# binbinmeng/QCNN_GPU

Measured on NVIDIA B200. Metric: luma Mpixel/s (QVRCNN int8, 1080p), higher is better.
Workload: dtype int8

## Files before the change

### include/qvrcnn_b200.h

```cpp
#ifndef QVRCNN_B200_H
#define QVRCNN_B200_H

#include <stddef.h>
#include <stdint.h>

#ifdef __cplusplus
extern "C" {
#endif

#if defined(__GNUC__)
#define QV_API __attribute__((visibility("default")))
#else
#define QV_API
#endif

typedef struct qv_net qv_net;

enum {
    QV_OK = 0,
    QV_ERR_ARG = -1,
    QV_ERR_IO = -2,
    QV_ERR_CUDA = -3,
    QV_ERR_RANGE = -4,
    QV_ERR_STATE = -5
};

enum {
    QV_IMPL_AUTO = 0,
    QV_IMPL_LAYERED = 1,
    QV_IMPL_FUSED = 2
};

enum { QV_C1 = 0, QV_C2_1 = 1, QV_C2_2 = 2, QV_C3_1 = 3, QV_C3_2 = 4, QV_C4 = 5, QV_NLAYER = 6 };

QV_API const char *qv_last_error(void);
QV_API const char *qv_version(void);


QV_API int qv_create(int gpu_num, int batch, int channel, int height, int width, qv_net **out);
QV_API int qv_destroy(qv_net *net);

QV_API int qv_load_static_para(qv_net *net, const char *filename);
QV_API int qv_load_static_para_mem(qv_net *net, const void *image, size_t len);
QV_API int qv_load_static_para_hwcn(qv_net *net, const char *filename);

QV_API int qv_load_quant_params(qv_net *net, const char *filename);
QV_API int qv_read_quant_params(const char *filename, int32_t *out18);
QV_API int qv_set_weights(qv_net *net, int layer, const int8_t *w_kcrs, const int32_t *bias);
QV_API int qv_get_quant_params(const qv_net *net, int32_t *out18);

QV_API int qv_load_data(qv_net *net, const uint8_t *host_luma);
QV_API int qv_forward_blu(qv_net *net);
QV_API int qv_get_recon(qv_net *net, uint8_t *host_out);

QV_API int qv_forward_frames_host(qv_net *net, const uint8_t *h_in, uint8_t *h_out, int n_frames);
QV_API int qv_stream_yuv(qv_net *net, const char *anchor_yuv, const char *ori_yuv, const char *recon_yuv,
                         int first_frame, int n_frames, int64_t *sse_before, int64_t *sse_after);
QV_API int qv_stream_yuv_pf(qv_net *net, const char *anchor_yuv, const char *ori_yuv, const char *recon_yuv,
                            int first_frame, int n_frames, int64_t *sse_before_pf, int64_t *sse_after_pf);
QV_API int qv_forward_frames_device(qv_net *net, const uint8_t *d_in, uint8_t *d_out, int n_frames,
                                    void *cuda_stream);
QV_API int qv_forward_frames_device_sse(qv_net *net, const uint8_t *d_in, const uint8_t *d_ori, uint8_t *d_out,
                                        int n_frames, int64_t *d_sse, void *cuda_stream);
QV_API int qv_forward_rows_device(qv_net *net, const uint8_t *d_in, int img_height, int in_row0, int in_rows,
                                  uint8_t *d_out, int out_row0, int out_row1, void *cuda_stream);

QV_API int qv_synchronize(qv_net *net, void *cuda_stream);

typedef struct { unsigned char opaque[192]; } qv_strip_desc;
enum { QV_STRIP_ABOVE = 0, QV_STRIP_BELOW = 1 };
QV_API int qv_strip_setup(qv_net *net, int img_height, int row0, int row1);
QV_API int qv_strip_export(qv_net *net, qv_strip_desc *out);
QV_API int qv_strip_attach(qv_net *net, int side, const qv_strip_desc *neighbour);
QV_API int qv_strip_input(qv_net *net, int slot, void **d_rows);
QV_API int qv_strip_acquire(qv_net *net, int slot, void *cuda_stream);
QV_API int qv_strip_load(qv_net *net, int slot, const uint8_t *host_rows, void *cuda_stream);
QV_API int qv_strip_forward(qv_net *net, int slot, uint8_t *d_out, void *cuda_stream);
QV_API int qv_strip_forward_sse(qv_net *net, int slot, const uint8_t *d_ori_rows, uint8_t *d_out, int64_t *d_sse2,
                                void *cuda_stream);
QV_API int qv_strip_release(qv_net *net);

QV_API int qv_device_buffers(qv_net *net, void **d_x, void **d_x_rec);

QV_API int qv_sse_device(const uint8_t *d_a, const uint8_t *d_b, size_t n, int64_t *d_sse_accum, void *cuda_stream);

QV_API int qv_set_impl(qv_net *net, int impl);
QV_API int qv_get_impl(const qv_net *net);
QV_API long long qv_launch_count(const qv_net *net);
QV_API int qv_get_activation(qv_net *net, int which , int8_t *host_out);

QV_API int qv_debug_fused_tables(const void *model_image, size_t len, uint8_t *wimg, uint32_t *ops, int32_t *consts, size_t sizes[3]);

QV_API int qv_debug_fused_units(int sm_count, int n_frames, int height, int width, int row0, int row1, int row_window, int allow_line,
                                int32_t *units, size_t *n_units, int *grid);

QV_API int qv_convert_model_hwcn_to_vect_c(const char *file_in, const char *file_out);

QV_API int qv_solve_quant_params(const double *stepw_in, const double *blu_in, double *rows_out36);
QV_API int qv_write_quant_params_cpp(const char *filename, const double *rows36);
QV_API int qv_quantize_layer(const float *w, size_t n_w, const float *b, size_t n_b, double stepw, double ratio,
                             int8_t *w_q, int32_t *b_q);

QV_API void *qv_host_alloc(size_t bytes);
QV_API void qv_host_free(void *p);

QV_API int qv_yuv_read_luma(const char *filename, int frames, int height, int width, uint8_t *out);
QV_API int qv_yuv_read_frame(const char *filename, int n, int height, int width, uint8_t *out);
QV_API int qv_yuv_write_recon(const char *filename, const uint8_t *luma, int frames, int height, int width);
QV_API double qv_psnr(const uint8_t *data, const uint8_t *ori, size_t n, int64_t *sse_out);
QV_API double qv_psnr_from_sse(int64_t sse, size_t n);

#ifdef __cplusplus
}
#endif
#endif
```

### qcnn_gpu_b200/api.py

```python
from __future__ import annotations

import ctypes as C
import os
from typing import Optional

import numpy as np

_PKG = os.path.dirname(os.path.abspath(__file__))
LIB_PATH = os.environ.get("QVRCNN_B200_LIB", os.path.join(_PKG, "libqvrcnn_b200.so"))

IMPL_AUTO, IMPL_LAYERED, IMPL_FUSED = 0, 1, 2

ABI_SYMBOLS = (
    "qv_last_error", "qv_version", "qv_create", "qv_destroy", "qv_load_static_para",
    "qv_load_static_para_mem", "qv_load_static_para_hwcn", "qv_load_quant_params", "qv_read_quant_params",
    "qv_set_weights", "qv_get_quant_params", "qv_load_data", "qv_forward_blu", "qv_get_recon",
    "qv_forward_frames_host", "qv_stream_yuv", "qv_stream_yuv_pf", "qv_forward_frames_device", "qv_forward_frames_device_sse", "qv_forward_rows_device", "qv_device_buffers",
    "qv_sse_device", "qv_host_alloc", "qv_host_free",
    "qv_set_impl", "qv_get_impl", "qv_launch_count", "qv_get_activation",
    "qv_convert_model_hwcn_to_vect_c", "qv_yuv_read_luma", "qv_yuv_read_frame", "qv_yuv_write_recon",
    "qv_psnr", "qv_psnr_from_sse", "qv_solve_quant_params", "qv_write_quant_params_cpp", "qv_quantize_layer",
    "qv_debug_fused_tables", "qv_debug_fused_units", "qv_synchronize",
    "qv_strip_setup", "qv_strip_export", "qv_strip_attach", "qv_strip_input", "qv_strip_acquire", "qv_strip_load",
    "qv_strip_forward", "qv_strip_forward_sse", "qv_strip_release",
)

CUDA_STREAM_LEGACY = 1
STRIP_ABOVE, STRIP_BELOW = 0, 1
STRIP_DESC_BYTES = 192


def stream_arg(stream: int):
    return CUDA_STREAM_LEGACY if not stream else stream


class QVError(RuntimeError):
    def __init__(self, code: int, msg: str):
        super().__init__("qvrcnn_b200 error %d: %s" % (code, msg))
        self.code = code


_lib = None


def lib():
    global _lib
    if _lib is None:
        if not os.path.exists(LIB_PATH):
            raise ImportError("%s not found: build it with `python -c 'import __graft_entry__ as g; g.build()'` "
                              "(there is no fallback implementation)" % LIB_PATH)
        L = C.CDLL(LIB_PATH)
        vp, i32, cp = C.c_void_p, C.c_int, C.c_char_p
        L.qv_last_error.restype = cp
        L.qv_version.restype = cp
        L.qv_create.argtypes = [i32, i32, i32, i32, i32, C.POINTER(vp)]
        L.qv_destroy.argtypes = [vp]
        L.qv_load_static_para.argtypes = [vp, cp]
        L.qv_load_static_para_mem.argtypes = [vp, vp, C.c_size_t]
        L.qv_load_static_para_hwcn.argtypes = [vp, cp]
        L.qv_load_quant_params.argtypes = [vp, cp]
        L.qv_read_quant_params.argtypes = [cp, vp]
        L.qv_set_weights.argtypes = [vp, i32, vp, vp]
        L.qv_get_quant_params.argtypes = [vp, vp]
        L.qv_load_data.argtypes = [vp, vp]
        L.qv_forward_blu.argtypes = [vp]
        L.qv_get_recon.argtypes = [vp, vp]
        L.qv_forward_frames_host.argtypes = [vp, vp, vp, i32]
        L.qv_forward_frames_device.argtypes = [vp, vp, vp, i32, vp]
        L.qv_forward_frames_device_sse.argtypes = [vp, vp, vp, vp, i32, vp, vp]
        L.qv_host_alloc.argtypes = [C.c_size_t]
        L.qv_host_alloc.restype = vp
        L.qv_host_free.argtypes = [vp]
        L.qv_host_free.restype = None
        L.qv_stream_yuv.argtypes = [vp, cp, cp, cp, i32, i32, C.POINTER(C.c_int64), C.POINTER(C.c_int64)]
        L.qv_stream_yuv_pf.argtypes = [vp, cp, cp, cp, i32, i32, vp, vp]
        L.qv_forward_rows_device.argtypes = [vp, vp, i32, i32, i32, vp, i32, i32, vp]
        L.qv_sse_device.argtypes = [vp, vp, C.c_size_t, vp, vp]
        L.qv_set_impl.argtypes = [vp, i32]
        L.qv_get_impl.argtypes = [vp]
        L.qv_launch_count.argtypes = [vp]
        L.qv_launch_count.restype = C.c_longlong
        L.qv_get_activation.argtypes = [vp, i32, vp]
        L.qv_convert_model_hwcn_to_vect_c.argtypes = [cp, cp]
        L.qv_yuv_read_luma.argtypes = [cp, i32, i32, i32, vp]
        L.qv_yuv_read_frame.argtypes = [cp, i32, i32, i32, vp]
        L.qv_yuv_write_recon.argtypes = [cp, vp, i32, i32, i32]
        L.qv_psnr.argtypes = [vp, vp, C.c_size_t, C.POINTER(C.c_int64)]
        L.qv_psnr.restype = C.c_double
        L.qv_psnr_from_sse.argtypes = [C.c_int64, C.c_size_t]
        L.qv_psnr_from_sse.restype = C.c_double
        L.qv_solve_quant_params.argtypes = [vp, vp, vp]
        L.qv_write_quant_params_cpp.argtypes = [cp, vp]
        L.qv_quantize_layer.argtypes = [vp, C.c_size_t, vp, C.c_size_t, C.c_double, C.c_double, vp, vp]
        L.qv_synchronize.argtypes = [vp, vp]
        L.qv_strip_setup.argtypes = [vp, i32, i32, i32]
        L.qv_strip_export.argtypes = [vp, vp]
        L.qv_strip_attach.argtypes = [vp, i32, vp]
        L.qv_strip_input.argtypes = [vp, i32, C.POINTER(vp)]
        L.qv_strip_acquire.argtypes = [vp, i32, vp]
        L.qv_strip_load.argtypes = [vp, i32, vp, vp]
        L.qv_strip_forward.argtypes = [vp, i32, vp, vp]
        L.qv_strip_forward_sse.argtypes = [vp, i32, vp, vp, vp, vp]
        L.qv_strip_release.argtypes = [vp]
        _lib = L
    return _lib


def _check(rc: int) -> None:
    if rc != 0:
        raise QVError(rc, lib().qv_last_error().decode("utf-8", "replace"))


def _b(path) -> bytes:
    return os.fsencode(path)


class QVRCNN:

    def __init__(self, gpu_num: int, batch: int, channel: int, height: int, width: int):
        self._h = C.c_void_p()
        self.batch, self.channel, self.height, self.width = batch, channel, height, width
        _check(lib().qv_create(gpu_num, batch, channel, height, width, C.byref(self._h)))

    def close(self) -> None:
        if getattr(self, "_h", None) and self._h.value:
            lib().qv_destroy(self._h)
            self._h = C.c_void_p()

    __del__ = close

    def load_static_para(self, filename) -> int:
        _check(lib().qv_load_static_para(self._h, _b(filename)))
        return 0

    def load_static_para_mem(self, image: bytes) -> int:
        _check(lib().qv_load_static_para_mem(self._h, image, len(image)))
        return 0

    def load_static_para_hwcn(self, filename) -> int:
        _check(lib().qv_load_static_para_hwcn(self._h, _b(filename)))
        return 0

    def load_quant_params(self, filename) -> int:
        _check(lib().qv_load_quant_params(self._h, _b(filename)))
        return 0

    def set_weights(self, layer: int, w_kcrs: np.ndarray, bias: np.ndarray) -> int:
        w = np.ascontiguousarray(w_kcrs, np.int8)
        b = np.ascontiguousarray(bias, np.int32)
        _check(lib().qv_set_weights(self._h, layer, w.ctypes.data, b.ctypes.data))
        return 0

    def quant_params(self) -> np.ndarray:
        q = np.zeros(18, np.int32)
        _check(lib().qv_get_quant_params(self._h, q.ctypes.data))
        return q.reshape(6, 3)

    def load_data(self, input_u8: np.ndarray) -> int:
        x = np.ascontiguousarray(input_u8, np.uint8)
        assert x.size == self.batch * self.height * self.width, x.shape
        _check(lib().qv_load_data(self._h, x.ctypes.data))
        return 0

    def forward_blu(self) -> int:
        _check(lib().qv_forward_blu(self._h))
        return 0

    def get_recon(self) -> np.ndarray:
        out = np.empty((self.batch, self.height, self.width), np.uint8)
        _check(lib().qv_get_recon(self._h, out.ctypes.data))
        return out

    def forward_frames_host(self, frames_u8: np.ndarray, out: Optional[np.ndarray] = None) -> np.ndarray:
        x = np.ascontiguousarray(frames_u8, np.uint8)
        n = x.size // (self.height * self.width)
        if out is None:
            out = np.empty_like(x)
        _check(lib().qv_forward_frames_host(self._h, x.ctypes.data, out.ctypes.data, n))
        return out

    def stream_yuv(self, anchor_yuv: str, ori_yuv: Optional[str], recon_yuv: Optional[str], first_frame: int, n_frames: int):
        b, a = C.c_int64(0), C.c_int64(0)
        enc = lambda p: p.encode() if p else None
        _check(lib().qv_stream_yuv(self._h, enc(anchor_yuv), enc(ori_yuv), enc(recon_yuv), first_frame, n_frames,
                                   C.byref(b) if ori_yuv else None, C.byref(a) if ori_yuv else None))
        return int(b.value), int(a.value)

    def stream_yuv_pf(self, anchor_yuv: str, ori_yuv: str, recon_yuv: Optional[str], first_frame: int, n_frames: int):
        before = np.zeros(max(n_frames, 0), np.int64)
        after = np.zeros(max(n_frames, 0), np.int64)
        enc = lambda p: os.fsencode(p) if p else None
        _check(lib().qv_stream_yuv_pf(self._h, enc(anchor_yuv), enc(ori_yuv), enc(recon_yuv), first_frame, n_frames,
                                      before.ctypes.data, after.ctypes.data))
        return before, after

    def forward_frames_host_ptr(self, in_ptr: int, out_ptr: int, n: int) -> None:
        _check(lib().qv_forward_frames_host(self._h, in_ptr, out_ptr, n))

    def forward_frames_device(self, d_in: int, d_out: int, n: int, stream: int = 0) -> None:
        _check(lib().qv_forward_frames_device(self._h, d_in, d_out, n, stream or None))

    def forward_frames_device_sse(self, d_in: int, d_ori: int, d_out: int, n: int, d_sse: int, stream: int = 0) -> None:
        _check(lib().qv_forward_frames_device_sse(self._h, d_in, d_ori, d_out, n, d_sse, stream or None))

    def forward_rows_device(self, d_in: int, img_height: int, in_row0: int, in_rows: int, d_out: int,
                            out_row0: int, out_row1: int, stream: int = 0) -> None:
        _check(lib().qv_forward_rows_device(self._h, d_in, img_height, in_row0, in_rows, d_out, out_row0,
                                            out_row1, stream or None))

    def synchronize(self, stream: int = 0) -> None:
        _check(lib().qv_synchronize(self._h, stream or None))

    def strip_setup(self, img_height: int, row0: int, row1: int) -> None:
        _check(lib().qv_strip_setup(self._h, img_height, row0, row1))
        self._strip_bytes = (row1 - row0) * self.width

    def strip_export(self) -> bytes:
        buf = C.create_string_buffer(STRIP_DESC_BYTES)
        _check(lib().qv_strip_export(self._h, buf))
        return buf.raw

    def strip_attach(self, side: int, desc: bytes) -> None:
        assert len(desc) == STRIP_DESC_BYTES
        _check(lib().qv_strip_attach(self._h, side, C.create_string_buffer(desc, STRIP_DESC_BYTES)))

    def strip_input(self, slot: int) -> int:
        p = C.c_void_p()
        _check(lib().qv_strip_input(self._h, slot, C.byref(p)))
        return int(p.value)

    def strip_acquire(self, slot: int, stream: int = 0) -> None:
        _check(lib().qv_strip_acquire(self._h, slot, stream or None))

    def strip_load(self, slot: int, rows_u8: np.ndarray, stream: int = 0) -> None:
        x = np.ascontiguousarray(rows_u8, np.uint8)
        assert x.size == getattr(self, "_strip_bytes", -1), "strip_load: expected the %d bytes of this handle's rows, got %d" % (getattr(self, "_strip_bytes", -1), x.size)
        _check(lib().qv_strip_load(self._h, slot, x.ctypes.data, stream or None))

    def strip_forward(self, slot: int, d_out: int, stream: int = 0) -> None:
        _check(lib().qv_strip_forward(self._h, slot, d_out, stream or None))

    def strip_forward_sse(self, slot: int, d_ori_rows: int, d_out: int, d_sse2: int, stream: int = 0) -> None:
        _check(lib().qv_strip_forward_sse(self._h, slot, d_ori_rows, d_out, d_sse2, stream or None))

    def strip_release(self) -> None:
        _check(lib().qv_strip_release(self._h))

    def set_impl(self, impl: int) -> None:
        _check(lib().qv_set_impl(self._h, impl))

    def get_impl(self) -> int:
        return lib().qv_get_impl(self._h)

    def launch_count(self) -> int:
        return int(lib().qv_launch_count(self._h))

    def get_activation(self, which: int) -> np.ndarray:
        out = np.empty((64 if which == 1 else 48, self.height, self.width), np.int8)
        _check(lib().qv_get_activation(self._h, which, out.ctypes.data))
        return out


def sse_device(d_a: int, d_b: int, n: int, d_accum: int, stream: int = 0) -> None:
    _check(lib().qv_sse_device(d_a, d_b, n, d_accum, stream or None))


def read_quant_params(filename) -> np.ndarray:
    q = np.zeros(18, np.int32)
    _check(lib().qv_read_quant_params(_b(filename), q.ctypes.data))
    return q.reshape(6, 3)


def convert_model_hwcn_to_vect_c(file_in, file_out) -> None:
    _check(lib().qv_convert_model_hwcn_to_vect_c(_b(file_in), _b(file_out)))


def solve_quant_params(stepw_in, blu_in) -> np.ndarray:
    a = np.ascontiguousarray(stepw_in, np.float64)
    b = np.ascontiguousarray(blu_in, np.float64)
    assert a.size == 6 and b.size == 6
    out = np.zeros(36, np.float64)
    _check(lib().qv_solve_quant_params(a.ctypes.data, b.ctypes.data, out.ctypes.data))
    return out.reshape(6, 6)


def write_quant_params_cpp(filename, rows) -> None:
    r = np.ascontiguousarray(rows, np.float64)
    assert r.size == 36
    _check(lib().qv_write_quant_params_cpp(_b(filename), r.ctypes.data))


def quantize_layer(w: np.ndarray, b: np.ndarray, stepw: float, ratio: float):
    wf = np.ascontiguousarray(w, np.float32)
    bf = np.ascontiguousarray(b, np.float32)
    wq = np.empty(wf.shape, np.int8)
    bq = np.empty(bf.shape, np.int32)
    _check(lib().qv_quantize_layer(wf.ctypes.data, wf.size, bf.ctypes.data, bf.size, float(stepw), float(ratio), wq.ctypes.data, bq.ctypes.data))
    return wq, bq


def psnr_from_sse(sse: int, n: int) -> float:
    return float(lib().qv_psnr_from_sse(sse, n))


class VRCNNData:

    def __init__(self, frame: int, height: int, width: int):
        self.frame, self.h, self.w = frame, height, width
        self.nSize = frame * height * width
        self.ori = np.zeros((frame, height, width), np.uint8)
        self.input = np.zeros((frame, height, width), np.uint8)
        self.recon = np.zeros((frame, height, width), np.uint8)

    def read_data(self, orifile, inputfile) -> int:
        _check(lib().qv_yuv_read_luma(_b(orifile), self.frame, self.h, self.w, self.ori.ctypes.data))
        _check(lib().qv_yuv_read_luma(_b(inputfile), self.frame, self.h, self.w, self.input.ctypes.data))
        return 0

    def read_frame(self, orifile, inputfile, n: int) -> int:
        self.frame = 1
        _check(lib().qv_yuv_read_frame(_b(orifile), n, self.h, self.w, self.ori.ctypes.data))
        _check(lib().qv_yuv_read_frame(_b(inputfile), n, self.h, self.w, self.input.ctypes.data))
        return 0

    def psnr(self, data: np.ndarray) -> float:
        d = np.ascontiguousarray(data, np.uint8)
        return float(lib().qv_psnr(d.ctypes.data, self.ori.ctypes.data, self.nSize, None))

    def save_recon_as(self, filename) -> int:
        _check(lib().qv_yuv_write_recon(_b(filename), self.recon.ctypes.data, self.frame, self.h, self.w))
        return 0
```

### qcnn_gpu_b200/csrc/qv_api.cu

```cuda
#include <algorithm>
#include <atomic>
#include <condition_variable>
#include <cstdio>
#include <cstdlib>
#include <cstring>
#include <mutex>
#include <random>
#include <thread>
#include <vector>

#include <fcntl.h>
#include <unistd.h>

#include <cuda_runtime.h>

#include "qv_fused.h"
#include "qv_internal.h"
#include "qv_layered.h"

using namespace qv;

#define QV_CUDA(expr)                                                                       \
    do {                                                                                    \
        cudaError_t e__ = (expr);                                                           \
        if (e__ != cudaSuccess) {                                                           \
            set_error("%s failed: %s (%s:%d)", #expr, cudaGetErrorString(e__), __FILE__, __LINE__); \
            return QV_ERR_CUDA;                                                             \
        }                                                                                   \
    } while (0)

namespace {
constexpr int STRIP_HALO = 6;
constexpr size_t STRIP_HDR = 256, STRIP_PUB = 0, STRIP_DONE = 64, STRIP_CTR = 128;
constexpr uint32_t STRIP_MAGIC = 0x51565354u;
struct StripDescImpl {
    uint32_t magic;
    int32_t dev, row0, row1, width, img_h;
    uint64_t nonce;
    uint64_t base, slot_off, slot_stride;
    uint64_t net;
    cudaIpcMemHandle_t ipc;
    char pci[16];
};
static_assert(sizeof(StripDescImpl) <= sizeof(qv_strip_desc), "qv_strip_desc too small");
struct StripPeer {
    bool attached = false, ipc = false, same_device = false;
    uint8_t *base = nullptr;
    qv_net *net = nullptr;
    StripDescImpl d{};
};
struct StripState {
    bool on = false;
    int img_h = 0, row0 = 0, row1 = 0;
    uint8_t *block = nullptr;
    size_t slot_stride = 0;
    uint32_t seq = 0, slot_seq[2] = {0, 0};
    uint32_t fills[2] = {0, 0}, forwards[2] = {0, 0};
    cudaStream_t last_stream = nullptr;
    bool used = false;
    StripPeer peer[2];
};
std::mutex g_strip_mu;
std::vector<qv_net *> g_strip_nets[64];
uint64_t process_nonce()
{
    static const uint64_t n = [] {
        std::random_device rd;
        return ((uint64_t)rd() << 32) ^ (uint64_t)rd() ^ ((uint64_t)getpid() << 17);
    }();
    return n;
}
}

struct qv_net {
    StripState strip;
    int dev = 0, batch = 0, H = 0, W = 0;
    cudaStream_t st = nullptr;
    cudaStream_t pst[2] = {nullptr, nullptr};
    cudaEvent_t ev_compute = nullptr;
    uint8_t *d_x = nullptr, *d_rec = nullptr;
    uint8_t *d_slot_in[2] = {nullptr, nullptr}, *d_slot_out[2] = {nullptr, nullptr};
    uint8_t *h_pin_in[2] = {nullptr, nullptr}, *h_pin_out[2] = {nullptr, nullptr};
    int8_t *d_a1 = nullptr, *d_a2 = nullptr, *d_a3 = nullptr;
    int act_frames = 0;
    uint8_t *d_rows_tmp = nullptr;
    size_t rows_tmp_bytes = 0;
    ModelHost model;
    LayeredModel lm;
    FusedModel *fm = nullptr;
    bool uploaded = false;
    int impl = QV_IMPL_AUTO;
    long long launches = 0;
};

static int set_device(const qv_net *net) { QV_CUDA(cudaSetDevice(net->dev)); return QV_OK; }

static void free_layered(qv_net *net)
{
    for (int l = 0; l < QV_NLAYER; ++l) {
        cudaFree(net->lm.L[l].d_wpk);
        cudaFree(net->lm.L[l].d_bias);
        net->lm.L[l].d_wpk = nullptr;
        net->lm.L[l].d_bias = nullptr;
    }
}

static inline int pack4(const int8_t *p, int stride, int n)
{
    int v = 0;
    for (int j = 0; j < n; ++j) v |= ((int)(uint8_t)p[j * stride]) << (8 * j);
    return v;
}

static int upload_layered(qv_net *net)
{
    free_layered(net);
    for (int l = 0; l < QV_NLAYER; ++l) {
        const LayerShape &s = kLayers[l];
        const LayerHost &L = net->model.L[l];
        std::vector<int32_t> wpk;
        const int R = s.k;
        if (l == QV_C1) {
            wpk.assign(5 * 64 * 2, 0);
            for (int r = 0; r < 5; ++r)
                for (int k = 0; k < 64; ++k) {
                    const int8_t *row = &L.w[((size_t)k * 5 + r) * 5];
                    wpk[(r * 64 + k) * 2 + 0] = pack4(row, 1, 4);
                    wpk[(r * 64 + k) * 2 + 1] = pack4(row + 4, 1, 1);
                }
        } else if (l == QV_C4) {
            wpk.assign(9 * 12, 0);
            for (int t = 0; t < 9; ++t)
                for (int c4 = 0; c4 < 12; ++c4)
                    wpk[t * 12 + c4] = pack4(&L.w[((size_t)(4 * c4) * 3 + t / 3) * 3 + t % 3], 9, 4);
        } else {
            const int C4 = s.cin / 4, G = s.cout / 16;
            wpk.assign((size_t)G * R * R * C4 * 16, 0);
            for (int g = 0; g < G; ++g)
                for (int t = 0; t < R * R; ++t)
                    for (int c4 = 0; c4 < C4; ++c4)
                        for (int j = 0; j < 16; ++j) {
                            const int k = g * 16 + j;
                            wpk[(((size_t)g * R * R + t) * C4 + c4) * 16 + j] =
                                pack4(&L.w[(((size_t)k * s.cin + 4 * c4) * R + t / R) * R + t % R], R * R, 4);
                        }
        }
        LayeredLayer &D = net->lm.L[l];
        D.cout = s.cout;
        D.q.blu = L.blu; D.q.mul = L.mul; D.q.shift = L.shift;
        D.q.rbias = (1 << (L.shift - 1)) / L.mul;
        QV_CUDA(cudaMalloc(&D.d_wpk, wpk.size() * sizeof(int32_t)));
        QV_CUDA(cudaMalloc(&D.d_bias, L.b.size() * sizeof(int32_t)));
        QV_CUDA(cudaMemcpyAsync(D.d_wpk, wpk.data(), wpk.size() * sizeof(int32_t), cudaMemcpyHostToDevice, net->st));
        QV_CUDA(cudaMemcpyAsync(D.d_bias, L.b.data(), L.b.size() * sizeof(int32_t), cudaMemcpyHostToDevice, net->st));
        QV_CUDA(cudaStreamSynchronize(net->st));
    }
    net->lm.c4_bias = net->model.L[QV_C4].b[0];
    return QV_OK;
}

static int validate_qparams(const ModelHost &m)
{
    for (int l = 0; l < QV_NLAYER; ++l) {
        const LayerHost &L = m.L[l];
        if (L.mul <= 0 || L.shift < 1 || L.shift > 30) {
            set_error("layer %d: mul=%d shift=%d outside the supported range (mul>0, 1<=shift<=30)", l, L.mul, L.shift);
            return QV_ERR_RANGE;
        }
        if (l != QV_C4 && (L.blu < 0 || L.blu >= (1 << 24))) {
            set_error("layer %d: blu=%d outside [0, 2^24)", l, L.blu);
            return QV_ERR_RANGE;
        }
    }
    return QV_OK;
}

static int sync_model(qv_net *net)
{
    net->uploaded = false;
    if (!net->model.complete()) return QV_OK;
    int rc = validate_qparams(net->model);
    if (rc) return rc;
    rc = check_fp32_exact_envelope(net->model);
    if (rc) return rc;
    if ((rc = set_device(net))) return rc;
    if ((rc = upload_layered(net))) return rc;
    if (net->fm) { fused_free(net->fm); net->fm = nullptr; }
    net->fm = fused_upload(net->model, net->st);
    net->uploaded = true;
    return QV_OK;
}

static int ensure_acts(qv_net *net)
{
    if (net->d_a1) return QV_OK;
    int frames = std::min(net->batch, 8);
    const size_t px = (size_t)frames * net->H * net->W;
    QV_CUDA(cudaMalloc(&net->d_a1, px * 64));
    QV_CUDA(cudaMalloc(&net->d_a2, px * 48));
    QV_CUDA(cudaMalloc(&net->d_a3, px * 48));
    net->act_frames = frames;
    return QV_OK;
}

static int run_forward(qv_net *net, const uint8_t *d_in, uint8_t *d_out, int n, int H, int W, cudaStream_t st,
                       const uint8_t *d_ori = nullptr, int64_t *d_sse = nullptr)
{
    if (!net->uploaded) {
        set_error("forward called before a complete model (weights + quant params) was loaded");
        return QV_ERR_STATE;
    }
    int impl = net->impl;
    if (impl == QV_IMPL_AUTO) impl = net->fm ? QV_IMPL_FUSED : QV_IMPL_LAYERED;
    if (impl == QV_IMPL_FUSED) {
        if (!net->fm) { set_error("fused tcgen05 path is not available in this build"); return QV_ERR_STATE; }
        if (d_sse && H > FUSED_SSE_MAX_H) { set_error("per-frame SSE: frame height %d exceeds %d", H, FUSED_SSE_MAX_H); return QV_ERR_ARG; }
        QV_CUDA(fused_forward(net->fm, d_in, d_out, n, H, W, st, &net->launches, nullptr, d_ori, d_sse));
        return QV_OK;
    }
    int rc = ensure_acts(net);
    if (rc) return rc;
    const size_t cap_px = (size_t)net->act_frames * net->H * net->W;
    const size_t fpx = (size_t)H * W;
    if (fpx > cap_px) { set_error("frame of %dx%d exceeds the handle's activation scratch", W, H); return QV_ERR_ARG; }
    const int chunk = (int)std::max<size_t>(1, cap_px / fpx);
    for (int f0 = 0; f0 < n; f0 += chunk) {
        const int c = std::min(chunk, n - f0);
        QV_CUDA(layered_forward(net->lm, d_in + (size_t)f0 * fpx, d_out + (size_t)f0 * fpx, c, H, W, net->d_a1,
                                net->d_a2, net->d_a3, st, &net->launches));
    }
    if (d_sse) {
        for (int f = 0; f < n; ++f) {
            const size_t o = (size_t)f * fpx;
            QV_CUDA(sse_accumulate(d_in + o, d_ori + o, fpx, d_sse + 2 * f, st));
            QV_CUDA(sse_accumulate(d_out + o, d_ori + o, fpx, d_sse + 2 * f + 1, st));
        }
        net->launches += 2 * n;
    }
    return QV_OK;
}

extern "C" {

int qv_create(int gpu_num, int batch, int channel, int height, int width, qv_net **out)
{
    if (!out) { set_error("qv_create: null output pointer"); return QV_ERR_ARG; }
    *out = nullptr;
    if (channel != 1) { set_error("qv_create: channel must be 1 (luma), got %d", channel); return QV_ERR_ARG; }
    if (batch < 1 || height < 1 || width < 1) { set_error("qv_create: bad geometry %dx%dx%d", batch, height, width); return QV_ERR_ARG; }
    int ndev = 0;
    if (cudaGetDeviceCount(&ndev) != cudaSuccess || ndev == 0) {
        set_error("qv_create: no CUDA device (this library has no CPU fallback)");
        return QV_ERR_CUDA;
    }
    if (gpu_num < 0 || gpu_num >= ndev) { set_error("qv_create: gpu_num %d out of range (%d devices)", gpu_num, ndev); return QV_ERR_ARG; }
    QV_CUDA(cudaSetDevice(gpu_num));
    qv_net *net = new qv_net();
    net->dev = gpu_num; net->batch = batch; net->H = height; net->W = width;
    const size_t bytes = (size_t)batch * height * width;
    cudaError_t e = cudaStreamCreateWithFlags(&net->st, cudaStreamNonBlocking);
    if (e == cudaSuccess) e = cudaMalloc(&net->d_x, bytes);
    if (e == cudaSuccess) e = cudaMalloc(&net->d_rec, bytes);
    if (e != cudaSuccess) {
        set_error("qv_create: %s", cudaGetErrorString(e));
        qv_destroy(net);
        return QV_ERR_CUDA;
    }
    *out = net;
    return QV_OK;
}

int qv_destroy(qv_net *net)
{
    if (!net) return QV_OK;
    cudaSetDevice(net->dev);
    if (net->st) cudaStreamSynchronize(net->st);
    qv_strip_release(net);
    free_layered(net);
    if (net->fm) fused_free(net->fm);
    cudaFree(net->d_x); cudaFree(net->d_rec);
    cudaFree(net->d_a1); cudaFree(net->d_a2); cudaFree(net->d_a3);
    cudaFree(net->d_rows_tmp);
    for (int i = 0; i < 2; ++i) {
        cudaFree(net->d_slot_in[i]); cudaFree(net->d_slot_out[i]);
        cudaFreeHost(net->h_pin_in[i]); cudaFreeHost(net->h_pin_out[i]);
        if (net->pst[i]) cudaStreamDestroy(net->pst[i]);
    }
    if (net->ev_compute) cudaEventDestroy(net->ev_compute);
    if (net->st) cudaStreamDestroy(net->st);
    delete net;
    return QV_OK;
}

int qv_load_static_para_mem(qv_net *net, const void *image, size_t len)
{
    if (!net || !image) { set_error("qv_load_static_para_mem: null argument"); return QV_ERR_ARG; }
    ModelHost m;
    int rc = parse_model_vect_c((const uint8_t *)image, len, m);
    if (rc) return rc;
    net->model = m;
    return sync_model(net);
}

int qv_debug_fused_tables(const void *image, size_t len, uint8_t *wimg, uint32_t *ops, int32_t *consts, size_t sizes[3])
{
    if (!image || !sizes) { set_error("qv_debug_fused_tables: null argument"); return QV_ERR_ARG; }
    ModelHost m;
    int rc = parse_model_vect_c((const uint8_t *)image, len, m);
    if (rc) return rc;
    std::vector<uint8_t> w;
    std::vector<uint32_t> o;
    std::vector<int32_t> c;
    fused_debug_tables(m, w, o, c);
    if (wimg && sizes[0] >= w.size()) memcpy(wimg, w.data(), w.size());
    if (ops && sizes[1] >= o.size()) memcpy(ops, o.data(), o.size() * sizeof(uint32_t));
    if (consts && sizes[2] >= c.size()) memcpy(consts, c.data(), c.size() * sizeof(int32_t));
    sizes[0] = w.size(); sizes[1] = o.size(); sizes[2] = c.size();
    return QV_OK;
}

int qv_debug_fused_units(int sm_count, int n_frames, int height, int width, int row0, int row1, int row_window, int allow_line,
                         int32_t *units, size_t *n_units, int *grid)
{
    if (!n_units || !grid) { set_error("qv_debug_fused_units: null argument"); return QV_ERR_ARG; }
    std::vector<int> u;
    int g = 0;
    if (fused_debug_units(sm_count, n_frames, height, width, row0, row1, row_window != 0, allow_line != 0, u, g)) {
        set_error("qv_debug_fused_units: bad geometry");
        return QV_ERR_ARG;
    }
    if (units && *n_units >= u.size() / 5) memcpy(units, u.data(), u.size() * sizeof(int));
    *n_units = u.size() / 5;
    *grid = g;
    return QV_OK;
}

int qv_load_static_para(qv_net *net, const char *filename)
{
    if (!net) { set_error("qv_load_static_para: null handle"); return QV_ERR_ARG; }
    std::vector<uint8_t> buf;
    int rc = read_file(filename, buf);
    if (rc) { set_error("cannot open model file. (%s)", filename ? filename : "(null)"); return rc; }
    return qv_load_static_para_mem(net, buf.data(), buf.size());
}

int qv_load_static_para_hwcn(qv_net *net, const char *filename)
{
    if (!net) { set_error("qv_load_static_para_hwcn: null handle"); return QV_ERR_ARG; }
    std::vector<uint8_t> buf;
    int rc = read_file(filename, buf);
    if (rc) return rc;
    ModelHost m;
    rc = parse_model_hwcn(buf.data(), buf.size(), m);
    if (rc) return rc;
    net->model = m;
    return sync_model(net);
}

int qv_load_quant_params(qv_net *net, const char *filename)
{
    if (!net) { set_error("qv_load_quant_params: null handle"); return QV_ERR_ARG; }
    int32_t q[18];
    int rc = qv_read_quant_params(filename, q);
    if (rc) return rc;
    for (int l = 0; l < QV_NLAYER; ++l) {
        LayerHost &L = net->model.L[l];
        L.blu = q[3 * l]; L.mul = q[3 * l + 1]; L.shift = q[3 * l + 2];
        L.have_q = true;
    }
    return sync_model(net);
}

int qv_set_weights(qv_net *net, int layer, const int8_t *w_kcrs, const int32_t *bias)
{
    if (!net || !w_kcrs || !bias || layer < 0 || layer >= QV_NLAYER) { set_error("qv_set_weights: bad argument"); return QV_ERR_ARG; }
    const LayerShape &s = kLayers[layer];
    LayerHost &L = net->model.L[layer];
    L.w.assign(w_kcrs, w_kcrs + (size_t)s.cout * s.cin * s.k * s.k);
    L.b.assign(bias, bias + s.cout);
    L.have_w = true;
    return sync_model(net);
}

int qv_get_quant_params(const qv_net *net, int32_t *out18)
{
    if (!net || !out18) { set_error("qv_get_quant_params: null argument"); return QV_ERR_ARG; }
    for (int l = 0; l < QV_NLAYER; ++l) {
        out18[3 * l] = net->model.L[l].blu; out18[3 * l + 1] = net->model.L[l].mul; out18[3 * l + 2] = net->model.L[l].shift;
    }
    return QV_OK;
}

int qv_load_data(qv_net *net, const uint8_t *host_luma)
{
    if (!net || !host_luma) { set_error("qv_load_data: null argument"); return QV_ERR_ARG; }
    int rc = set_device(net);
    if (rc) return rc;
    const size_t bytes = (size_t)net->batch * net->H * net->W;
    QV_CUDA(cudaMemcpyAsync(net->d_x, host_luma, bytes, cudaMemcpyHostToDevice, net->st));
    QV_CUDA(cudaStreamSynchronize(net->st));
    return QV_OK;
}

static int kernel_report(qv_net *net)
{
    const int f = net->fm ? fused_take_failure(net->fm) : 0;
    if (!f) return QV_OK;
    set_error(f == 2 ? "fused kernel: a CTA saw other shared-memory / TMEM bases than the operand table was built for"
              : f == 3 ? "strip mode: a neighbour GPU's rows were never published (the frame data of this call is not valid)"
                       : "fused kernel: an mbarrier wait timed out (the frame data of this call is not valid)");
    return QV_ERR_CUDA;
}

int qv_forward_blu(qv_net *net)
{
    if (!net) { set_error("qv_forward_blu: null handle"); return QV_ERR_ARG; }
    int rc = set_device(net);
    if (rc) return rc;
    rc = run_forward(net, net->d_x, net->d_rec, net->batch, net->H, net->W, net->st);
    if (rc) return rc;
    QV_CUDA(cudaStreamSynchronize(net->st));
    return kernel_report(net);
}

int qv_get_recon(qv_net *net, uint8_t *host_out)
{
    if (!net || !host_out) { set_error("qv_get_recon: null argument"); return QV_ERR_ARG; }
    int rc = set_device(net);
    if (rc) return rc;
    const size_t bytes = (size_t)net->batch * net->H * net->W;
    QV_CUDA(cudaMemcpyAsync(host_out, net->d_rec, bytes, cudaMemcpyDeviceToHost, net->st));
    QV_CUDA(cudaStreamSynchronize(net->st));
    return kernel_report(net);
}

int qv_forward_frames_device(qv_net *net, const uint8_t *d_in, uint8_t *d_out, int n_frames, void *cuda_stream)
{
    if (!net || !d_in || !d_out || n_frames < 0) { set_error("qv_forward_frames_device: bad argument"); return QV_ERR_ARG; }
    int rc = set_device(net);
    if (rc) return rc;
    cudaStream_t st = cuda_stream ? (cudaStream_t)cuda_stream : net->st;
    if (n_frames > 0) {
        rc = run_forward(net, d_in, d_out, n_frames, net->H, net->W, st);
        if (rc) return rc;
    }
    if (!cuda_stream) { QV_CUDA(cudaStreamSynchronize(st)); return kernel_report(net); }
    return QV_OK;
}

int qv_forward_frames_device_sse(qv_net *net, const uint8_t *d_in, const uint8_t *d_ori, uint8_t *d_out, int n_frames,
                                 int64_t *d_sse, void *cuda_stream)
{
    if (!net || !d_in || !d_ori || !d_out || !d_sse || n_frames < 0) { set_error("qv_forward_frames_device_sse: bad argument"); return QV_ERR_ARG; }
    int rc = set_device(net);
    if (rc) return rc;
    cudaStream_t st = cuda_stream ? (cudaStream_t)cuda_stream : net->st;
    if (n_frames > 0) {
        rc = run_forward(net, d_in, d_out, n_frames, net->H, net->W, st, d_ori, d_sse);
        if (rc) return rc;
    }
    if (!cuda_stream) { QV_CUDA(cudaStreamSynchronize(st)); return kernel_report(net); }
    return QV_OK;
}

int qv_forward_rows_device(qv_net *net, const uint8_t *d_in, int img_height, int in_row0, int in_rows, uint8_t *d_out,
                           int out_row0, int out_row1, void *cuda_stream)
{
    if (!net || !d_in || !d_out) { set_error("qv_forward_rows_device: null argument"); return QV_ERR_ARG; }
    const int in_row1 = in_row0 + in_rows;
    if (img_height < 1 || in_row0 < 0 || in_rows < 1 || in_row1 > img_height || out_row0 < in_row0 || out_row1 > in_row1 ||
        out_row0 > out_row1) { set_error("qv_forward_rows_device: inconsistent row ranges"); return QV_ERR_ARG; }
    if ((in_row0 != 0 && out_row0 - in_row0 < STRIP_HALO) || (in_row1 != img_height && in_row1 - out_row1 < STRIP_HALO)) {
        set_error("qv_forward_rows_device: need 6 halo rows on every interior strip edge");
        return QV_ERR_ARG;
    }
    int rc = set_device(net);
    if (rc) return rc;
    cudaStream_t st = cuda_stream ? (cudaStream_t)cuda_stream : net->st;
    const size_t W = net->W;
    const bool fused_path = net->impl == QV_IMPL_FUSED || (net->impl == QV_IMPL_AUTO && net->fm);
    if (fused_path) {
        if (!net->uploaded || !net->fm) { set_error("forward called before a complete model (weights + quant params) was loaded"); return QV_ERR_STATE; }
        FusedRows fr;
        fr.own0 = in_row0; fr.own1 = in_row1; fr.out0 = out_row0; fr.out1 = out_row1;
        QV_CUDA(fused_forward(net->fm, d_in, d_out, 1, img_height, net->W, st, &net->launches, &fr));
    } else {
        const size_t need = (size_t)in_rows * W;
        if (need > (size_t)net->batch * net->H * net->W) {
            set_error("qv_forward_rows_device: window larger than the handle's geometry");
            return QV_ERR_ARG;
        }
        if (net->rows_tmp_bytes < need) {
            QV_CUDA(cudaStreamSynchronize(st));
            cudaFree(net->d_rows_tmp);
            net->d_rows_tmp = nullptr; net->rows_tmp_bytes = 0;
            QV_CUDA(cudaMalloc(&net->d_rows_tmp, need));
            net->rows_tmp_bytes = need;
        }
        rc = run_forward(net, d_in, net->d_rows_tmp, 1, in_rows, net->W, st);
        if (rc) return rc;
        QV_CUDA(cudaMemcpyAsync(d_out, net->d_rows_tmp + (size_t)(out_row0 - in_row0) * W, (size_t)(out_row1 - out_row0) * W,
                                cudaMemcpyDeviceToDevice, st));
    }
    if (!cuda_stream) { QV_CUDA(cudaStreamSynchronize(st)); return kernel_report(net); }
    return QV_OK;
}

int qv_synchronize(qv_net *net, void *cuda_stream)
{
    if (!net) { set_error("qv_synchronize: null handle"); return QV_ERR_ARG; }
    int rc = set_device(net);
    if (rc) return rc;
    QV_CUDA(cudaStreamSynchronize(cuda_stream ? (cudaStream_t)cuda_stream : net->st));
    return kernel_report(net);
}

static void strip_detach(qv_net *net)
{
    for (StripPeer &p : net->strip.peer) {
        if (p.attached && p.ipc && p.base) cudaIpcCloseMemHandle(p.base);
        p = StripPeer{};
    }
}

int qv_strip_release(qv_net *net)
{
    if (!net) { set_error("qv_strip_release: null handle"); return QV_ERR_ARG; }
    if (!net->strip.on) return QV_OK;
    cudaSetDevice(net->dev);
    cudaStreamSynchronize(net->st);
    strip_detach(net);
    cudaFree(net->strip.block);
    net->strip = StripState{};
    if (net->dev >= 0 && net->dev < 64) {
        std::lock_guard<std::mutex> l(g_strip_mu);
        auto &v = g_strip_nets[net->dev];
        v.erase(std::remove(v.begin(), v.end(), net), v.end());
    }
    return QV_OK;
}

int qv_strip_setup(qv_net *net, int img_height, int row0, int row1)
{
    if (!net) { set_error("qv_strip_setup: null handle"); return QV_ERR_ARG; }
    if (img_height < 1 || row0 < 0 || row1 <= row0 || row1 > img_height) { set_error("qv_strip_setup: rows [%d, %d) of %d", row0, row1, img_height); return QV_ERR_ARG; }
    int rc = set_device(net);
    if (rc) return rc;
    qv_strip_release(net);
    StripState &S = net->strip;
    S.img_h = img_height; S.row0 = row0; S.row1 = row1;
    S.slot_stride = ((size_t)(row1 - row0) * net->W + 255) / 256 * 256;
    QV_CUDA(cudaMalloc(&S.block, STRIP_HDR + 2 * S.slot_stride));
    QV_CUDA(cudaMemset(S.block, 0, STRIP_HDR));
    QV_CUDA(cudaDeviceSynchronize());
    S.on = true;
    if (net->dev >= 0 && net->dev < 64) {
        std::lock_guard<std::mutex> l(g_strip_mu);
        g_strip_nets[net->dev].push_back(net);
    }
    return QV_OK;
}

int qv_strip_export(qv_net *net, qv_strip_desc *out)
{
    if (!net || !out) { set_error("qv_strip_export: null argument"); return QV_ERR_ARG; }
    if (!net->strip.on) { set_error("qv_strip_export: qv_strip_setup has not been called"); return QV_ERR_STATE; }
    int rc = set_device(net);
    if (rc) return rc;
    StripDescImpl d{};
    d.magic = STRIP_MAGIC; d.dev = net->dev; d.row0 = net->strip.row0; d.row1 = net->strip.row1; d.width = net->W; d.img_h = net->strip.img_h;
    d.nonce = process_nonce();
    d.base = (uint64_t)(uintptr_t)net->strip.block; d.slot_off = STRIP_HDR; d.slot_stride = net->strip.slot_stride;
    d.net = (uint64_t)(uintptr_t)net;
    QV_CUDA(cudaIpcGetMemHandle(&d.ipc, net->strip.block));
    QV_CUDA(cudaDeviceGetPCIBusId(d.pci, (int)sizeof(d.pci), net->dev));
    memset(out, 0, sizeof(*out));
    memcpy(out, &d, sizeof(d));
    return QV_OK;
}

int qv_strip_attach(qv_net *net, int side, const qv_strip_desc *neighbour)
{
    if (!net || !neighbour || (side != QV_STRIP_ABOVE && side != QV_STRIP_BELOW)) { set_error("qv_strip_attach: bad argument"); return QV_ERR_ARG; }
    StripState &S = net->strip;
    if (!S.on) { set_error("qv_strip_attach: qv_strip_setup has not been called"); return QV_ERR_STATE; }
    StripDescImpl d;
    memcpy(&d, neighbour, sizeof(d));
    if (d.magic != STRIP_MAGIC) { set_error("qv_strip_attach: not a strip descriptor"); return QV_ERR_ARG; }
    if (d.width != net->W || d.img_h != S.img_h) { set_error("qv_strip_attach: the neighbour's frame is %dx%d, this one %dx%d", d.width, d.img_h, net->W, S.img_h); return QV_ERR_ARG; }
    if (side == QV_STRIP_ABOVE ? d.row1 != S.row0 : d.row0 != S.row1) {
        set_error("qv_strip_attach: rows [%d, %d) are not adjacent %s rows [%d, %d)", d.row0, d.row1, side == QV_STRIP_ABOVE ? "above" : "below", S.row0, S.row1);
        return QV_ERR_ARG;
    }
    if (d.row1 - d.row0 < STRIP_HALO) {
        set_error("qv_strip_attach: the neighbour holds %d rows, fewer than the %d-row halo (use fewer strips)", d.row1 - d.row0, STRIP_HALO);
        return QV_ERR_ARG;
    }
    int rc = set_device(net);
    if (rc) return rc;
    StripPeer &P = S.peer[side];
    if (P.attached && P.ipc && P.base) cudaIpcCloseMemHandle(P.base);
    P = StripPeer{};
    if (d.nonce == process_nonce()) {
        if (d.dev != net->dev) {
            int can = 0;
            QV_CUDA(cudaDeviceCanAccessPeer(&can, net->dev, d.dev));
            if (!can) { set_error("qv_strip_attach: device %d cannot map memory of device %d (no peer access)", net->dev, d.dev); return QV_ERR_CUDA; }
            cudaError_t e = cudaDeviceEnablePeerAccess(d.dev, 0);
            if (e == cudaErrorPeerAccessAlreadyEnabled) { cudaGetLastError(); e = cudaSuccess; }
            QV_CUDA(e);
        }
        P.base = (uint8_t *)(uintptr_t)d.base;
        P.net = (qv_net *)(uintptr_t)d.net;
    } else {
        char my_pci[16] = {0};
        QV_CUDA(cudaDeviceGetPCIBusId(my_pci, (int)sizeof(my_pci), net->dev));
        if (strncmp(my_pci, d.pci, sizeof(my_pci)) == 0) {
            set_error("qv_strip_attach: the neighbour strip belongs to another process on the SAME GPU; strips of different processes must be on different GPUs");
            return QV_ERR_ARG;
        }
        void *p = nullptr;
        QV_CUDA(cudaIpcOpenMemHandle(&p, d.ipc, cudaIpcMemLazyEnablePeerAccess));
        P.base = (uint8_t *)p;
        P.ipc = true;
    }
    P.d = d;
    char my_pci[16] = {0};
    QV_CUDA(cudaDeviceGetPCIBusId(my_pci, (int)sizeof(my_pci), net->dev));
    P.same_device = strncmp(my_pci, d.pci, sizeof(my_pci)) == 0;
    P.attached = true;
    return QV_OK;
}

int qv_strip_input(qv_net *net, int slot, void **d_rows)
{
    if (!net || !d_rows || slot < 0 || slot > 1) { set_error("qv_strip_input: bad argument"); return QV_ERR_ARG; }
    if (!net->strip.on) { set_error("qv_strip_input: qv_strip_setup has not been called"); return QV_ERR_STATE; }
    *d_rows = net->strip.block + STRIP_HDR + (size_t)slot * net->strip.slot_stride;
    return QV_OK;
}

static int check_shared_device_stream(qv_net *net, cudaStream_t st, const char *who)
{
    std::lock_guard<std::mutex> l(g_strip_mu);
    for (qv_net *o : g_strip_nets[net->dev])
        if (o != net && o->strip.used && o->strip.last_stream != st) {
            set_error("%s: several strips live on GPU %d: drive all of them on ONE caller-provided stream (kernels of different launches "
                      "must not wait for each other on one GPU, so stream order is what orders them)", who, net->dev);
            return QV_ERR_STATE;
        }
    return QV_OK;
}

int qv_strip_acquire(qv_net *net, int slot, void *cuda_stream)
{
    if (!net || slot < 0 || slot > 1) { set_error("qv_strip_acquire: bad argument"); return QV_ERR_ARG; }
    StripState &S = net->strip;
    if (!S.on) { set_error("qv_strip_acquire: qv_strip_setup has not been called"); return QV_ERR_STATE; }
    int rc = set_device(net);
    if (rc) return rc;
    cudaStream_t st = cuda_stream ? (cudaStream_t)cuda_stream : net->st;
    if ((rc = check_shared_device_stream(net, st, "qv_strip_acquire"))) return rc;
    S.last_stream = st; S.used = true;
    const uint32_t s = S.slot_seq[slot];
    const uint32_t *w[2] = {nullptr, nullptr};
    for (int side = 0; side < 2; ++side) {
        const StripPeer &P = S.peer[side];
        if (!P.attached || s == 0) continue;
        if (P.same_device) {
            if (P.net->strip.forwards[slot] < S.forwards[slot]) {
                set_error("qv_strip_acquire: the neighbour strip on the same GPU has not yet consumed slot %d (issue the strips' calls frame by frame)", slot);
                return QV_ERR_STATE;
            }
        } else {
            w[side] = reinterpret_cast<const uint32_t *>(P.base + STRIP_DONE);
        }
    }
    if (net->fm && (w[0] || w[1])) {
        QV_CUDA(fused_wait_words(net->fm, w[0], s, w[1], s, st));
        net->launches += 1;
    }
    S.fills[slot] += 1;
    return QV_OK;
}

int qv_strip_load(qv_net *net, int slot, const uint8_t *host_rows, void *cuda_stream)
{
    if (!host_rows) { set_error("qv_strip_load: null argument"); return QV_ERR_ARG; }
    int rc = qv_strip_acquire(net, slot, cuda_stream);
    if (rc) return rc;
    StripState &S = net->strip;
    QV_CUDA(cudaMemcpyAsync(S.block + STRIP_HDR + (size_t)slot * S.slot_stride, host_rows, (size_t)(S.row1 - S.row0) * net->W,
                            cudaMemcpyHostToDevice, cuda_stream ? (cudaStream_t)cuda_stream : net->st));
    return QV_OK;
}

static int strip_forward(qv_net *net, int slot, const uint8_t *d_ori, uint8_t *d_out, int64_t *d_sse, void *cuda_stream, const char *who)
{
    StripState &S = net->strip;
    if (!S.on) { set_error("%s: qv_strip_setup has not been called", who); return QV_ERR_STATE; }
    if (!net->uploaded || !net->fm || net->impl == QV_IMPL_LAYERED) {
        set_error("%s: needs a loaded model and the fused path (peer-mapped halo rows are read by the fused kernel)", who);
        return QV_ERR_STATE;
    }
    if ((S.row0 > 0 && !S.peer[QV_STRIP_ABOVE].attached) || (S.row1 < S.img_h && !S.peer[QV_STRIP_BELOW].attached)) {
        set_error("%s: rows [%d, %d) of %d have an interior edge with no neighbour attached", who, S.row0, S.row1, S.img_h);
        return QV_ERR_STATE;
    }
    if (d_sse && S.img_h > FUSED_SSE_MAX_H) { set_error("%s: frame height %d exceeds %d", who, S.img_h, FUSED_SSE_MAX_H); return QV_ERR_ARG; }
    int rc = set_device(net);
    if (rc) return rc;
    cudaStream_t st = cuda_stream ? (cudaStream_t)cuda_stream : net->st;
    if ((rc = check_shared_device_stream(net, st, who))) return rc;
    const size_t W = net->W;
    FusedRows fr;
    fr.own0 = fr.out0 = S.row0; fr.own1 = fr.out1 = S.row1;
    fr.pub = reinterpret_cast<uint32_t *>(S.block + STRIP_PUB);
    fr.done = reinterpret_cast<uint32_t *>(S.block + STRIP_DONE);
    fr.done_ctr = reinterpret_cast<uint32_t *>(S.block + STRIP_CTR);
    for (int side = 0; side < 2; ++side) {
        if (side == QV_STRIP_ABOVE ? S.row0 == 0 : S.row1 == S.img_h) continue;
        const StripPeer &P = S.peer[side];
        const uint8_t *rows = P.base + P.d.slot_off + (size_t)slot * P.d.slot_stride;
        const uint32_t *flag = reinterpret_cast<const uint32_t *>(P.base + STRIP_PUB);
        if (P.same_device) {
            if (P.net->strip.fills[slot] == 0) {
                set_error("%s: the neighbour strip on the same GPU has not filled slot %d yet (strips that share a GPU: all loads of a frame, then its forwards, on one stream)", who, slot);
                return QV_ERR_STATE;
            }
            flag = nullptr;
        }
        if (side == QV_STRIP_ABOVE) { fr.top_rows = STRIP_HALO; fr.d_top = rows + (size_t)(P.d.row1 - P.d.row0 - STRIP_HALO) * W; fr.flag_top = flag; }
        else { fr.bot_rows = STRIP_HALO; fr.d_bot = rows; fr.flag_bot = flag; }
    }
    const uint32_t seq = ++S.seq;
    S.slot_seq[slot] = seq;
    S.forwards[slot] += 1;
    S.last_stream = st; S.used = true;
    fr.seq = seq;
    const uint8_t *own = S.block + STRIP_HDR + (size_t)slot * S.slot_stride;
    QV_CUDA(fused_forward(net->fm, own, d_out, 1, S.img_h, net->W, st, &net->launches, &fr, d_ori, d_sse));
    if (!cuda_stream) { QV_CUDA(cudaStreamSynchronize(st)); return kernel_report(net); }
    return QV_OK;
}

int qv_strip_forward(qv_net *net, int slot, uint8_t *d_out, void *cuda_stream)
{
    if (!net || !d_out || slot < 0 || slot > 1) { set_error("qv_strip_forward: bad argument"); return QV_ERR_ARG; }
    return strip_forward(net, slot, nullptr, d_out, nullptr, cuda_stream, "qv_strip_forward");
}

int qv_strip_forward_sse(qv_net *net, int slot, const uint8_t *d_ori_rows, uint8_t *d_out, int64_t *d_sse2, void *cuda_stream)
{
    if (!net || !d_ori_rows || !d_out || !d_sse2 || slot < 0 || slot > 1) { set_error("qv_strip_forward_sse: bad argument"); return QV_ERR_ARG; }
    return strip_forward(net, slot, d_ori_rows, d_out, d_sse2, cuda_stream, "qv_strip_forward_sse");
}

int qv_forward_frames_host(qv_net *net, const uint8_t *h_in, uint8_t *h_out, int n_frames)
{
    if (!net || !h_in || !h_out || n_frames < 0) { set_error("qv_forward_frames_host: bad argument"); return QV_ERR_ARG; }
    int rc = set_device(net);
    if (rc) return rc;
    const size_t fpx = (size_t)net->H * net->W;
    std::vector<int> chunks;
    {
        static const int num[10] = {1, 3, 4, 8, 16, 16, 8, 4, 3, 1};
        int left = n_frames;
        if (n_frames >= 16) {
            for (int k = 0; k < 10 && left > 0; ++k) {
                int want = k == 9 ? left : std::max(1, n_frames * num[k] / 64);
                while (want > 0 && left > 0) {
                    const int c = std::min(std::min(want, left), net->batch);
                    chunks.push_back(c); want -= c; left -= c;
                }
            }
        }
        const char *ov = getenv("QV_E2E_CHUNKS");
        if (ov && *ov) {
            chunks.clear(); left = n_frames;
            for (const char *p = ov; *p && left > 0;) {
                const int c = std::min(std::min(std::max(1, atoi(p)), left), net->batch);
                chunks.push_back(c); left -= c;
                while (*p && *p != ',') ++p;
                if (*p == ',') ++p;
            }
        }
        const int uni = std::max(1, std::min(net->batch, (n_frames + 3) / 4));
        while (left > 0) { const int c = std::min(uni, left); chunks.push_back(c); left -= c; }
    }
    const size_t cbytes = (size_t)net->batch * fpx;
    cudaPointerAttributes ai{}, ao{};
    bool pinned_in = cudaPointerGetAttributes(&ai, h_in) == cudaSuccess && ai.type == cudaMemoryTypeHost;
    bool pinned_out = cudaPointerGetAttributes(&ao, h_out) == cudaSuccess && ao.type == cudaMemoryTypeHost;
    cudaGetLastError();
    if (!net->ev_compute) QV_CUDA(cudaEventCreateWithFlags(&net->ev_compute, cudaEventDisableTiming));
    for (int i = 0; i < 2; ++i) {
        if (!net->pst[i]) QV_CUDA(cudaStreamCreateWithFlags(&net->pst[i], cudaStreamNonBlocking));
        if (!net->d_slot_in[i]) QV_CUDA(cudaMalloc(&net->d_slot_in[i], cbytes));
        if (!net->d_slot_out[i]) QV_CUDA(cudaMalloc(&net->d_slot_out[i], cbytes));
        if (!pinned_in && !net->h_pin_in[i]) QV_CUDA(cudaMallocHost(&net->h_pin_in[i], cbytes));
        if (!pinned_out && !net->h_pin_out[i]) QV_CUDA(cudaMallocHost(&net->h_pin_out[i], cbytes));
    }
    struct Pending { int f0 = -1, c = 0; } pend[2];
    auto drain = [&](int s) -> int {
        if (pend[s].f0 < 0) return QV_OK;
        QV_CUDA(cudaStreamSynchronize(net->pst[s]));
        if (!pinned_out) memcpy(h_out + (size_t)pend[s].f0 * fpx, net->h_pin_out[s], (size_t)pend[s].c * fpx);
        pend[s].f0 = -1;
        return QV_OK;
    };
    int slot = 0;
    int f0 = 0;
    for (size_t ci = 0; ci < chunks.size(); f0 += chunks[ci], ++ci, slot ^= 1) {
        const int c = chunks[ci];
        const size_t bytes = (size_t)c * fpx;
        if ((rc = drain(slot))) return rc;
        const uint8_t *src = h_in + (size_t)f0 * fpx;
        if (!pinned_in) { memcpy(net->h_pin_in[slot], src, bytes); src = net->h_pin_in[slot]; }
        QV_CUDA(cudaMemcpyAsync(net->d_slot_in[slot], src, bytes, cudaMemcpyHostToDevice, net->pst[slot]));
        const bool fused_path = net->impl == QV_IMPL_FUSED || (net->impl == QV_IMPL_AUTO && net->fm);
        if (f0 > 0 && !fused_path) QV_CUDA(cudaStreamWaitEvent(net->pst[slot], net->ev_compute, 0));
        rc = run_forward(net, net->d_slot_in[slot], net->d_slot_out[slot], c, net->H, net->W, net->pst[slot]);
        if (rc) return rc;
        QV_CUDA(cudaEventRecord(net->ev_compute, net->pst[slot]));
        uint8_t *dst = pinned_out ? h_out + (size_t)f0 * fpx : net->h_pin_out[slot];
        QV_CUDA(cudaMemcpyAsync(dst, net->d_slot_out[slot], bytes, cudaMemcpyDeviceToHost, net->pst[slot]));
        pend[slot].f0 = f0; pend[slot].c = c;
    }
    if ((rc = drain(0))) return rc;
    if ((rc = drain(1))) return rc;
    return kernel_report(net);
}

namespace {
struct StreamSlot {
    uint8_t *h_in = nullptr, *h_ori = nullptr, *h_out = nullptr;
    uint8_t *d_in = nullptr, *d_ori = nullptr, *d_out = nullptr;
    cudaStream_t st = nullptr;
    cudaEvent_t done = nullptr;
    int state = 0;
    int f0 = 0, c = 0;
};
struct StreamShared {
    std::mutex mu;
    std::condition_variable cv;
    bool failed = false;
    char msg[256] = {0};
    void fail(const char *m) { std::lock_guard<std::mutex> l(mu); if (!failed) { failed = true; snprintf(msg, sizeof(msg), "%s", m); } cv.notify_all(); }
};
bool read_luma(FILE *f, long long frame, size_t fpx, uint8_t *dst)
{
    if (fseeko(f, (off_t)(frame * (long long)(fpx + fpx / 2)), SEEK_SET) != 0) return false;
    return fread(dst, 1, fpx, f) == fpx;
}
}

int qv_stream_yuv_pf(qv_net *net, const char *anchor_yuv, const char *ori_yuv, const char *recon_yuv, int first_frame, int n_frames,
                     int64_t *sse_before_pf, int64_t *sse_after_pf)
{
    if (!net || !anchor_yuv || first_frame < 0 || n_frames < 0) { set_error("qv_stream_yuv_pf: bad argument"); return QV_ERR_ARG; }
    if ((sse_before_pf || sse_after_pf) && !ori_yuv) { set_error("qv_stream_yuv_pf: an SSE was asked for but no original file given"); return QV_ERR_ARG; }
    int rc = set_device(net);
    if (rc) return rc;
    for (int j = 0; j < n_frames; ++j) {
        if (sse_before_pf) sse_before_pf[j] = 0;
        if (sse_after_pf) sse_after_pf[j] = 0;
    }
    if (n_frames == 0) return QV_OK;
    const size_t fpx = (size_t)net->H * net->W;
    const int C = net->batch, NS = 3;
    FILE *fa = fopen(anchor_yuv, "rb"), *fo = ori_yuv ? fopen(ori_yuv, "rb") : nullptr, *fr = nullptr;
    if (!fa) { set_error("open file failed. (%s)", anchor_yuv); return QV_ERR_IO; }
    if (ori_yuv && !fo) { fclose(fa); set_error("open file failed. (%s)", ori_yuv); return QV_ERR_IO; }
    if (recon_yuv) {
        const int fd = open(recon_yuv, O_CREAT | O_RDWR, 0644);
        fr = fd >= 0 ? fdopen(fd, "r+b") : nullptr;
        if (!fr && fd >= 0) close(fd);
        if (!fr) { fclose(fa); if (fo) fclose(fo); set_error("open file failed. (%s)", recon_yuv); return QV_ERR_IO; }
    }
    StreamSlot slot[3];
    StreamShared sh;
    int64_t *d_sse = nullptr;
    const size_t sse_bytes = (size_t)n_frames * 2 * sizeof(int64_t);
    cudaError_t e = cudaMalloc(&d_sse, sse_bytes);
    if (e == cudaSuccess) e = cudaMemset(d_sse, 0, sse_bytes);
    for (int s = 0; s < NS && e == cudaSuccess; ++s) {
        StreamSlot &S = slot[s];
        e = cudaMallocHost(&S.h_in, C * fpx);
        if (e == cudaSuccess) e = cudaMallocHost(&S.h_out, C * fpx);
        if (e == cudaSuccess && fo) e = cudaMallocHost(&S.h_ori, C * fpx);
        if (e == cudaSuccess) e = cudaMalloc(&S.d_in, C * fpx);
        if (e == cudaSuccess) e = cudaMalloc(&S.d_out, C * fpx);
        if (e == cudaSuccess && fo) e = cudaMalloc(&S.d_ori, C * fpx);
        if (e == cudaSuccess) e = cudaStreamCreateWithFlags(&S.st, cudaStreamNonBlocking);
        if (e == cudaSuccess) e = cudaEventCreateWithFlags(&S.done, cudaEventDisableTiming);
    }
    const int nchunk = (n_frames + C - 1) / C;
    auto cleanup = [&]() {
        for (int s = 0; s < NS; ++s) {
            StreamSlot &S = slot[s];
            if (S.st) cudaStreamSynchronize(S.st);
            cudaFreeHost(S.h_in); cudaFreeHost(S.h_out); cudaFreeHost(S.h_ori);
            cudaFree(S.d_in); cudaFree(S.d_out); cudaFree(S.d_ori);
            if (S.done) cudaEventDestroy(S.done);
            if (S.st) cudaStreamDestroy(S.st);
        }
        cudaFree(d_sse);
        fclose(fa); if (fo) fclose(fo); if (fr) fclose(fr);
    };
    if (e != cudaSuccess) { cleanup(); set_error("qv_stream_yuv: %s", cudaGetErrorString(e)); return QV_ERR_CUDA; }

    std::thread reader([&] {
        for (int k = 0; k < nchunk; ++k) {
            StreamSlot &S = slot[k % NS];
            {
                std::unique_lock<std::mutex> l(sh.mu);
                sh.cv.wait(l, [&] { return S.state == 0 || sh.failed; });
                if (sh.failed) return;
            }
            const int f0 = k * C, c = std::min(C, n_frames - f0);
            for (int j = 0; j < c; ++j) {
                if (!read_luma(fa, (long long)first_frame + f0 + j, fpx, S.h_in + (size_t)j * fpx) ||
                    (fo && !read_luma(fo, (long long)first_frame + f0 + j, fpx, S.h_ori + (size_t)j * fpx))) {
                    sh.fail("qv_stream_yuv: short read (file smaller than the requested frame range)");
                    return;
                }
            }
            { std::lock_guard<std::mutex> l(sh.mu); S.f0 = f0; S.c = c; S.state = 1; }
            sh.cv.notify_all();
        }
    });
    const int dev = net->dev;
    std::thread writer([&] {
        cudaSetDevice(dev);
        std::vector<uint8_t> zeros(fpx / 2, 0);
        for (int k = 0; k < nchunk; ++k) {
            StreamSlot &S = slot[k % NS];
            {
                std::unique_lock<std::mutex> l(sh.mu);
                sh.cv.wait(l, [&] { return S.state == 2 || sh.failed; });
                if (sh.failed) return;
            }
            if (cudaEventSynchronize(S.done) != cudaSuccess) { sh.fail("qv_stream_yuv: the GPU stage failed"); return; }
            if (fr) {
                bool ok = fseeko(fr, (off_t)(((long long)first_frame + S.f0) * (long long)(fpx + fpx / 2)), SEEK_SET) == 0;
                for (int j = 0; j < S.c && ok; ++j)
                    ok = fwrite(S.h_out + (size_t)j * fpx, 1, fpx, fr) == fpx && fwrite(zeros.data(), 1, fpx / 2, fr) == fpx / 2;
                if (!ok) { sh.fail("qv_stream_yuv: write to the reconstruction file failed"); return; }
            }
            { std::lock_guard<std::mutex> l(sh.mu); S.state = 0; }
            sh.cv.notify_all();
        }
    });
    const bool fused_path = net->impl == QV_IMPL_FUSED || (net->impl == QV_IMPL_AUTO && net->fm);
    cudaEvent_t ev_compute = nullptr;
    if (!fused_path && cudaEventCreateWithFlags(&ev_compute, cudaEventDisableTiming) != cudaSuccess) {
        sh.fail("qv_stream_yuv: the GPU stage failed");
        rc = QV_ERR_CUDA;
    }
    for (int k = 0; k < nchunk && rc == QV_OK; ++k) {
        StreamSlot &S = slot[k % NS];
        {
            std::unique_lock<std::mutex> l(sh.mu);
            sh.cv.wait(l, [&] { return S.state == 1 || sh.failed; });
            if (sh.failed) break;
        }
        const size_t bytes = (size_t)S.c * fpx;
        e = cudaMemcpyAsync(S.d_in, S.h_in, bytes, cudaMemcpyHostToDevice, S.st);
        if (e == cudaSuccess && fo) e = cudaMemcpyAsync(S.d_ori, S.h_ori, bytes, cudaMemcpyHostToDevice, S.st);
        if (e == cudaSuccess && !fused_path && k > 0) e = cudaStreamWaitEvent(S.st, ev_compute, 0);
        if (e == cudaSuccess) {
            rc = run_forward(net, S.d_in, S.d_out, S.c, net->H, net->W, S.st, fo ? S.d_ori : nullptr, fo ? d_sse + 2 * (size_t)S.f0 : nullptr);
            if (rc == QV_OK && !fused_path) e = cudaEventRecord(ev_compute, S.st);
        }
        if (e == cudaSuccess && rc == QV_OK) e = cudaMemcpyAsync(S.h_out, S.d_out, bytes, cudaMemcpyDeviceToHost, S.st);
        if (e == cudaSuccess && rc == QV_OK) e = cudaEventRecord(S.done, S.st);
        if (e != cudaSuccess) { set_error("qv_stream_yuv: %s", cudaGetErrorString(e)); rc = QV_ERR_CUDA; }
        if (rc != QV_OK) { sh.fail("qv_stream_yuv: the GPU stage failed"); break; }
        { std::lock_guard<std::mutex> l(sh.mu); S.state = 2; }
        sh.cv.notify_all();
    }
    reader.join();
    writer.join();
    if (ev_compute) { for (int s = 0; s < NS; ++s) cudaStreamSynchronize(slot[s].st); cudaEventDestroy(ev_compute); }
    std::vector<int64_t> h_sse(fo ? (size_t)n_frames * 2 : 0);
    if (rc == QV_OK && !sh.failed) {
        for (int s = 0; s < NS; ++s) cudaStreamSynchronize(slot[s].st);
        if (fo && cudaMemcpy(h_sse.data(), d_sse, sse_bytes, cudaMemcpyDeviceToHost) != cudaSuccess) {
            set_error("qv_stream_yuv_pf: copy of the SSEs failed");
            rc = QV_ERR_CUDA;
        }
    }
    cleanup();
    if (rc == QV_OK && sh.failed) { set_error("%s", sh.msg); rc = strstr(sh.msg, "GPU") ? QV_ERR_CUDA : QV_ERR_IO; }
    if (rc != QV_OK) return rc;
    for (int j = 0; fo && j < n_frames; ++j) {
        if (sse_before_pf) sse_before_pf[j] = h_sse[2 * (size_t)j];
        if (sse_after_pf) sse_after_pf[j] = h_sse[2 * (size_t)j + 1];
    }
    return kernel_report(net);
}

int qv_stream_yuv(qv_net *net, const char *anchor_yuv, const char *ori_yuv, const char *recon_yuv, int first_frame, int n_frames,
                  int64_t *sse_before, int64_t *sse_after)
{
    if (!net || !anchor_yuv || first_frame < 0 || n_frames < 0) { set_error("qv_stream_yuv: bad argument"); return QV_ERR_ARG; }
    if ((sse_before || sse_after) && !ori_yuv) { set_error("qv_stream_yuv: an SSE was asked for but no original file given"); return QV_ERR_ARG; }
    std::vector<int64_t> before(ori_yuv ? n_frames : 0), after(ori_yuv ? n_frames : 0);
    const int rc = qv_stream_yuv_pf(net, anchor_yuv, ori_yuv, recon_yuv, first_frame, n_frames, ori_yuv ? before.data() : nullptr,
                                    ori_yuv ? after.data() : nullptr);
    if (sse_before) *sse_before = 0;
    if (sse_after) *sse_after = 0;
    if (rc != QV_OK) return rc;
    for (size_t j = 0; j < before.size(); ++j) {
        if (sse_before) *sse_before += before[j];
        if (sse_after) *sse_after += after[j];
    }
    return QV_OK;
}

void *qv_host_alloc(size_t bytes)
{
    if (bytes == 0) bytes = 1;
    void *p = nullptr;
    int ndev = 0;
    if (cudaGetDeviceCount(&ndev) == cudaSuccess && ndev > 0 && cudaHostAlloc(&p, bytes, cudaHostAllocPortable) == cudaSuccess) return p;
    cudaGetLastError();
    return malloc(bytes);
}

void qv_host_free(void *p)
{
    if (!p) return;
    cudaPointerAttributes a{};
    if (cudaPointerGetAttributes(&a, p) == cudaSuccess && a.type == cudaMemoryTypeHost) { cudaFreeHost(p); return; }
    cudaGetLastError();
    free(p);
}

int qv_device_buffers(qv_net *net, void **d_x, void **d_x_rec)
{
    if (!net) { set_error("qv_device_buffers: null handle"); return QV_ERR_ARG; }
    if (d_x) *d_x = net->d_x;
    if (d_x_rec) *d_x_rec = net->d_rec;
    return QV_OK;
}

int qv_sse_device(const uint8_t *d_a, const uint8_t *d_b, size_t n, int64_t *d_sse_accum, void *cuda_stream)
{
    if (!d_a || !d_b || !d_sse_accum) { set_error("qv_sse_device: null argument"); return QV_ERR_ARG; }
    if (n == 0) return QV_OK;
    QV_CUDA(sse_accumulate(d_a, d_b, n, d_sse_accum, (cudaStream_t)cuda_stream));
    return QV_OK;
}

int qv_set_impl(qv_net *net, int impl)
{
    if (!net || impl < QV_IMPL_AUTO || impl > QV_IMPL_FUSED) { set_error("qv_set_impl: bad argument"); return QV_ERR_ARG; }
    net->impl = impl;
    return QV_OK;
}

int qv_get_impl(const qv_net *net)
{
    if (!net) return QV_ERR_ARG;
    if (net->impl != QV_IMPL_AUTO) return net->impl;
    return net->fm ? QV_IMPL_FUSED : QV_IMPL_LAYERED;
}

long long qv_launch_count(const qv_net *net) { return net ? net->launches : 0; }

int qv_get_activation(qv_net *net, int which, int8_t *host_out)
{
    if (!net || !host_out || which < 1 || which > 3) { set_error("qv_get_activation: bad argument"); return QV_ERR_ARG; }
    if (!net->d_a1) { set_error("qv_get_activation: the layered path has not run on this handle"); return QV_ERR_STATE; }
    int rc = set_device(net);
    if (rc) return rc;
    const int C = which == 1 ? 64 : 48;
    const int8_t *src = which == 1 ? net->d_a1 : (which == 2 ? net->d_a2 : net->d_a3);
    const size_t HW = (size_t)net->H * net->W;
    int8_t *tmp = nullptr;
    QV_CUDA(cudaMalloc(&tmp, HW * C));
    cudaError_t e = nhwc_to_planar(src, tmp, C, HW, net->st);
    if (e == cudaSuccess) e = cudaMemcpyAsync(host_out, tmp, HW * C, cudaMemcpyDeviceToHost, net->st);
    if (e == cudaSuccess) e = cudaStreamSynchronize(net->st);
    cudaFree(tmp);
    QV_CUDA(e);
    return QV_OK;
}

}
```

### qcnn_gpu_b200/csrc/qv_fused.cu

```cuda
#include <algorithm>
#include <cstdio>
#include <cstdlib>
#include <cstring>
#include <mutex>
#include <type_traits>
#include <vector>

#include <cuda.h>
#include <cuda_runtime.h>

#include "qv_device.cuh"
#include "qv_fused.h"
#include "qv_tcgen05.cuh"


#ifndef QV_EXP
#define QV_EXP 0
#endif
#ifndef QV_CODE_SHIFT
#define QV_CODE_SHIFT 5
#endif
#ifndef QV_SHIFT_WORK
#define QV_SHIFT_WORK 0
#endif
#ifndef QV_SHIFT_C4
#define QV_SHIFT_C4 0
#endif
#ifndef QV_BULK_WEIGHTS
#define QV_BULK_WEIGHTS 1
#endif
#ifndef QV_LIGHT_PROF
#define QV_LIGHT_PROF 0
#endif

namespace qv {
namespace {
using namespace tc;
constexpr int EXP = QV_EXP;

constexpr int WT = 120;
constexpr int PW = 136;
constexpr int PLANE = PW * 16;
constexpr int A_SLOTS = 3, IN_SLOTS = 32, IN_PITCH = 144;
constexpr int A1_ROW = 4 * PLANE, A2_ROW = 3 * PLANE;
constexpr int IM_BYTES = 2 * 128 * 16;
constexpr int ZERO_BYTES = 2 * 128 * 16;

constexpr int NR22 = 11 * 16, NR21 = 7 * 32, NR31 = 7 * 16, NR32 = 32;
constexpr int W1_BYTES = 2 * 64 * 16;
constexpr int T22 = 2 * NR22 * 16, T21 = 2 * NR21 * 16, T31 = 2 * NR31 * 16, T32 = 2 * NR32 * 16;
constexpr int OFF_W1 = 0;
constexpr int OFF_W22 = OFF_W1 + W1_BYTES;
constexpr int OFF_W21 = OFF_W22 + 10 * T22;
constexpr int OFF_W31 = OFF_W21 + 6 * T21;
constexpr int OFF_W32 = OFF_W31 + 5 * T31;
constexpr int OFF_BIAS = OFF_W32 + 2 * T32;
constexpr int BIAS_INTS = 64 + 48 + 48;
constexpr int WIMG_BYTES = OFF_BIAS + BIAS_INTS * 4;
constexpr int OFF_A1 = (WIMG_BYTES + 127) / 128 * 128;
constexpr int OFF_A2 = OFF_A1 + A_SLOTS * A1_ROW;
constexpr int OFF_IM = OFF_A2 + A_SLOTS * A2_ROW;
constexpr int OFF_ZERO = OFF_IM + 3 * IM_BYTES;
constexpr int OFF_IN = OFF_ZERO + ZERO_BYTES;
constexpr int OFF_A3 = (OFF_IN + IN_SLOTS * IN_PITCH + 15) / 16 * 16;
constexpr int OFF_CTRL = OFF_A3 + A_SLOTS * A2_ROW;
constexpr int SMEM_BYTES = OFF_CTRL + 64;
static_assert(SMEM_BYTES <= 232448, "exceeds the 227 KB of dynamic shared memory per CTA");
constexpr int IN_PITCH_T = 256, IN_BOX = 144;
constexpr int OFF_IN_T = (SMEM_BYTES + 127) / 128 * 128;
constexpr int SMEM_BYTES_T = OFF_IN_T + IN_SLOTS * IN_PITCH_T;
static_assert(SMEM_BYTES_T <= 232448, "exceeds the 227 KB of dynamic shared memory per CTA");

#ifndef QV_ONE_WORKER
#define QV_ONE_WORKER 1
#endif
constexpr int NWORKER = QV_ONE_WORKER ? 128 : 256, NC4 = 128, NTHREADS = NWORKER + 32 + NC4;
constexpr int MMA_WARP = NWORKER / 32;
constexpr int TR_ITER0 = 300, TR_N = 8;
constexpr int PIPE = 14;

constexpr int TM_D1 = 0;
constexpr int TM_R22 = 128;
constexpr int TM_R21 = 224;
constexpr int TM_R31 = 352;
constexpr int TM_D32 = 416;
constexpr int TM_COLS = 512;

struct GroupQ {
    int hi;
    unsigned M;
    int blu, mul, shift, rbias;
};

struct alignas(64) FusedParams {
    CUtensorMap tmap_in;
    const uint8_t *in;
    uint8_t *out;
    const uint8_t *wimg;
    int n_frames, H, W, nstrips, nseg, seg_rows, n_units, linear, perm_q, perm_s0, perm_r;
    int ys, ye, own0, own1, rlo, rhi;
    size_t frame_stride;
    const uint8_t *in_top, *in_bot;
    const uint32_t *flag_top, *flag_bot;
    uint32_t *pub, *done, *done_ctr;
    uint32_t seq;
    GroupQ q1, q22, q21, q31, q32;
    int c4_bias, c4_mul, c4_shift;
    int c4_w[108];
    long long *dbg;
    uint32_t sbase16, tmem_base;
    int *fail_flag;
    int dbg_flags;
    int bias[BIAS_INTS];
    const uint8_t *ori;
    unsigned long long *sse;
};

struct PhaseBases {
    uint32_t im, a1_r2, a2_r6, b22;
    uint32_t b21, b31, d1, d32;
    uint32_t z22, z21, z31, pad;
};
struct FixedBases { uint32_t zeroA, w1, w32, r22, r21, r31, pad0, pad1; };
constexpr int N_PHASE = 12;
constexpr int N_MMA = 27;
struct PhaseOps {
    uint4 ab[N_MMA];
    uint32_t d1, d32, z22, z21, z31, pad[3];
};
__constant__ PhaseOps c_ops[N_PHASE];

__host__ __device__ __forceinline__ int mod_pos(int a, int m) { int r = a % m; return r < 0 ? r + m : r; }

__host__ __device__ __forceinline__ int wrap_sub(int c, int k, int n) { const int v = c - (k % n); return v < 0 ? v + n : v; }
__host__ __device__ __forceinline__ int wrap_inc(int c, int n) { return c + 1 == n ? 0 : c + 1; }

__device__ __forceinline__ void warp_wait(uint64_t *bar, uint32_t parity, int lane, int *fail)
{
    if (lane == 0 && !tc::mbar_wait(bar, parity)) *fail = 1;
    __syncwarp();
}

__device__ __forceinline__ bool peer_wait(const uint32_t *flag, uint32_t seq)
{
    for (int n = 0; n < 4000000; ++n) {
        uint32_t v;
        asm volatile("ld.acquire.sys.global.u32 %0, [%1];" : "=r"(v) : "l"(flag) : "memory");
        if ((int)(v - seq) >= 0) return true;
        __nanosleep(200);
    }
    return false;
}

struct UnitGeo { int strip, f, y0, y1; bool ok; };
template <bool ROWS>
__host__ __device__ __forceinline__ UnitGeo unit_geo(const FusedParams &P, int unit, int H, int grid)
{
    UnitGeo g;
    if (!ROWS && P.linear) {
        const int b = unit % grid, j = unit / grid;
        const int lo = b * P.seg_rows, hi = min(P.n_frames * P.nstrips * H, lo + P.seg_rows), c = lo / H + j;
        const int start = j == 0 ? lo : c * H, end = min(hi, (c + 1) * H);
        const int full = P.perm_r * (P.perm_s0 + 1);
        const int q = c < full ? c / (P.perm_s0 + 1) : P.perm_r + (c - full) / P.perm_s0;
        const int sl = c < full ? c - q * (P.perm_s0 + 1) : (c - full) - (q - P.perm_r) * P.perm_s0;
        const int col = q + sl * P.perm_q;
        g.f = col / P.nstrips;
        g.strip = col - g.f * P.nstrips;
        g.y0 = start - c * H;
        g.y1 = g.y0 + (end - start);
        g.ok = start < end;
    } else if (!ROWS) {
        const int seg = unit % P.nseg;
        g.strip = (unit / P.nseg) % P.nstrips;
        g.f = unit / (P.nseg * P.nstrips);
        g.y0 = seg * P.seg_rows;
        g.y1 = min(H, g.y0 + P.seg_rows);
        g.ok = true;
    } else {
        const int R = P.ye - P.ys, b = unit % grid, j = unit / grid;
        const int lo = b * P.seg_rows, hi = min(P.nstrips * R, lo + P.seg_rows), c0 = lo / R;
        const int start = j == 0 ? lo : (c0 + j) * R, end = min(hi, (c0 + j + 1) * R);
        g.strip = c0 + j;
        g.f = 0;
        g.y0 = P.ys + (start - g.strip * R);
        g.y1 = g.y0 + (end - start);
        g.ok = start < end;
    }
    return g;
}

__device__ __forceinline__ void work_arrive(uint32_t ev)
{
    asm volatile("bar.arrive %0, %1;" ::"r"(2u + ev % 3u), "n"(NWORKER + NC4 + 32) : "memory");
}

template <bool FAST, int BOFF>
__device__ __forceinline__ void requant(const uint32_t (&r)[16], const FusedParams &P, const GroupQ &g, bool valid,
                                        uint32_t (&o)[4])
{
    const unsigned Mz = valid ? g.M : 0u;
#pragma unroll
    for (int v = 0; v < 4; ++v) {
        const int bb[4] = {P.bias[BOFF + 4 * v], P.bias[BOFF + 4 * v + 1], P.bias[BOFF + 4 * v + 2], P.bias[BOFF + 4 * v + 3]};
        uint32_t q[4];
#pragma unroll
        for (int j = 0; j < 4; ++j) {
            if (FAST) {
                const unsigned t = (unsigned)__viaddmin_s32_relu((int)r[4 * v + j], bb[j], g.hi);
                q[j] = t * Mz;
            } else {
                QParam qp{g.blu, g.mul, g.shift, g.rbias};
                q[j] = valid ? ((unsigned)blu_requant((int)r[4 * v + j] + bb[j], qp) << 24) : 0u;
            }
        }
        o[v] = __byte_perm(__byte_perm(q[0], q[1], 0x0073), __byte_perm(q[2], q[3], 0x0073), 0x5410);
    }
}
template <bool FAST, int BOFF>
__device__ __forceinline__ void requant_store(const uint32_t (&r)[16], const FusedParams &P, const GroupQ &g, bool valid,
                                              uint8_t *dst)
{
    uint32_t o[4];
    if (EXP & 2) { o[0] = r[0] & 0x7f7f7f7fu; o[1] = r[5] & 0x7f7f7f7fu; o[2] = r[10] & 0x7f7f7f7fu; o[3] = r[15] & 0x7f7f7f7fu; }
    else requant<FAST, BOFF>(r, P, g, valid, o);
    *reinterpret_cast<uint4 *>(dst) = make_uint4(o[0], o[1], o[2], o[3]);
}
template <int DX>
__device__ __forceinline__ void c4_taps(const uint4 (&v)[3], const FusedParams &P, int (&acc)[3])
{
#pragma unroll
    for (int dy = 0; dy < 3; ++dy)
#pragma unroll
        for (int pl = 0; pl < 3; ++pl) {
            const int *w = &P.c4_w[((dy * 3 + DX) * 3 + pl) * 4];
            acc[dy] = __dp4a((int)v[pl].x, w[0], acc[dy]);
            acc[dy] = __dp4a((int)v[pl].y, w[1], acc[dy]);
            acc[dy] = __dp4a((int)v[pl].z, w[2], acc[dy]);
            acc[dy] = __dp4a((int)v[pl].w, w[3], acc[dy]);
        }
}

template <bool FAST, bool PROF, bool ROWS, bool TMA = false>
__global__ void __launch_bounds__(NTHREADS, 1) k_fused(const __grid_constant__ FusedParams P)
{
    constexpr bool SSE = false;
#include "qv_fused_body.inc"
}

template <bool FAST, bool ROWS>
__global__ void __launch_bounds__(NTHREADS, 1) k_enh_sse(const __grid_constant__ FusedParams P)
{
    constexpr bool SSE = true, PROF = false, TMA = false;
#include "qv_fused_body.inc"
}

__global__ void k_wait_words(const uint32_t *a, uint32_t va, const uint32_t *b, uint32_t vb, int *fail_flag)
{
    const uint32_t *w = threadIdx.x == 0 ? a : b;
    const uint32_t v = threadIdx.x == 0 ? va : vb;
    if (w && !peer_wait(w, v)) { *reinterpret_cast<volatile int *>(fail_flag) = 3; __threadfence_system(); }
}

__global__ void k_bases(uint32_t *out)
{
    extern __shared__ __align__(1024) uint8_t sm[];
    uint32_t *slot = reinterpret_cast<uint32_t *>(sm);
    tmem_alloc(slot, TM_COLS);
    tmem_relinquish();
    fence_before_sync();
    __syncwarp();
    fence_after_sync();
    const uint32_t tm = *slot;
    if (threadIdx.x == 0) { out[0] = smem_u32(sm); out[1] = tm; }
    __syncwarp();
    tmem_dealloc(tm, TM_COLS);
}

void build_mma_bases(uint32_t sb, uint32_t tm, PhaseBases *pb, FixedBases &fb)
{
    constexpr uint32_t LP = (uint32_t)(PLANE >> 4) << 16;
    const uint32_t w22 = sb + (OFF_W22 >> 4) + ((uint32_t)NR22 << 16), w21 = sb + (OFF_W21 >> 4) + ((uint32_t)NR21 << 16);
    const uint32_t w31 = sb + (OFF_W31 >> 4) + ((uint32_t)NR31 << 16);
    fb = FixedBases{};
    fb.zeroA = sb + (OFF_ZERO >> 4) + ((128u * 16 >> 4) << 16);
    fb.w1 = sb + (OFF_W1 >> 4) + (64u << 16);
    fb.w32 = sb + (OFF_W32 >> 4) + ((uint32_t)NR32 << 16);
    fb.r22 = tm + TM_R22; fb.r21 = tm + TM_R21; fb.r31 = tm + TM_R31;
    for (int ph = 0; ph < N_PHASE; ++ph) {
        const int R1p = ph + 4096 / N_PHASE * N_PHASE + N_PHASE, c3 = ph % 3, c6 = ph % 6;
        const uint32_t par = ph & 1;
        const int qa = wrap_sub(c6, 2, 6);
        PhaseBases &e = pb[ph];
        e = PhaseBases{};
        e.im = sb + ((OFF_IM + c3 * IM_BYTES) >> 4) + ((128u * 16 >> 4) << 16);
        e.a1_r2 = sb + (OFF_A1 >> 4) + wrap_sub(c3, 2, 3) * (A1_ROW >> 4) + LP;
        e.a2_r6 = sb + (OFF_A2 >> 4) + c3 * (A2_ROW >> 4);
        e.b22 = w22 + (qa <= 2 ? 2 - qa : 8 - qa) * 16;
        e.b21 = w21 + ((1 - (R1p - 2)) & 3) * 32;
        e.b31 = w31 + ((1 - (R1p - 6)) & 3) * 16;
        e.d1 = tm + TM_D1 + par * 64; e.d32 = tm + TM_D32 + par * 32;
        e.z22 = tm + TM_R22 + c6 * 16;
        e.z21 = tm + TM_R21 + ((R1p - 1) & 3) * 32;
        e.z31 = tm + TM_R31 + ((R1p - 5) & 3) * 16;
    }
}

void build_mma_ops(const PhaseBases *pb, const FixedBases &fb, PhaseOps *ops)
{
    constexpr uint32_t HI = (128u >> 4) | (1u << 14);
    constexpr uint32_t LP = (uint32_t)(PLANE >> 4) << 16, LX = 1u << 16;
    for (int ph = 0; ph < N_PHASE; ++ph) {
        const PhaseBases &e = pb[ph];
        PhaseOps &o = ops[ph];
        o = PhaseOps{};
        int k = 0;
        auto put = [&](uint32_t a, uint32_t b) { o.ab[k++] = make_uint4(a, HI, b, HI); };
        put(e.im, fb.w1);
        put(fb.zeroA, fb.w1); put(fb.zeroA, fb.w1); put(fb.zeroA, fb.w1);
        put(e.a2_r6 + 6 + LP, e.b31);
        put(e.a2_r6 + 7 + LP, e.b31 + (T31 >> 4));
        put(e.a2_r6 + 7 + LP, fb.w32);
        put(e.a2_r6 + 8 + LP, e.b31 + 2 * (T31 >> 4));
        put(e.a2_r6 + ((2 * PLANE) >> 4) + 6 + LX, e.b31 + 3 * (T31 >> 4));
        put(e.a2_r6 + ((2 * PLANE) >> 4) + 6 + LX, fb.w32 + (T32 >> 4));
        put(e.a2_r6 + ((2 * PLANE) >> 4) + 8 + LX, e.b31 + 4 * (T31 >> 4));
        for (int t = 0; t < 10; ++t) {
            const int sft = t / 2, h = t & 1;
            const uint32_t a = e.a1_r2 + ((h * 2 * PLANE + (4 + sft) * 16) >> 4);
            put(a, e.b22 + t * (T22 >> 4));
            if (sft >= 1 && sft <= 3) put(a, e.b21 + ((sft - 1) * 2 + h) * (T21 >> 4));
        }
        o.d1 = e.d1; o.d32 = e.d32; o.z22 = e.z22; o.z21 = e.z21; o.z31 = e.z31;
    }
}

}

struct FusedModel {
    int *h_fail = nullptr;
    uint8_t *d_wimg = nullptr;
    FusedParams proto{};
    bool fast = true;
    int sm_count = 148;
    bool env_profile = false, env_test_fail = false, env_tma = false, env_linear = true;
    int env_experiment = 0;
    void *encode_tiled = nullptr;
};

static std::mutex g_ops_mu;
struct OpsRecord { bool done = false; uint32_t sbase16 = 0, tmem_base = 0; };
static OpsRecord g_ops_done[64];

static void put_chunk(uint8_t *blk, int NR, int j, int n, const int8_t *src16) { memcpy(blk + ((size_t)j * NR + n) * 16, src16, 16); }

static bool build_host_image(const ModelHost &m, std::vector<uint8_t> &img, FusedParams &P)
{
    img.assign(WIMG_BYTES, 0);
    auto Wt = [&](int l, int k, int c, int r, int s) -> int8_t {
        const LayerShape &sh = kLayers[l];
        return m.L[l].w[(((size_t)k * sh.cin + c) * sh.k + r) * sh.k + s];
    };
    for (int n = 0; n < 64; ++n) {
        int8_t k32[32] = {0};
        for (int r = 0; r < 5; ++r) {
            for (int s = 0; s < 4; ++s) k32[4 * r + s] = Wt(QV_C1, n, 0, r, s);
            k32[20 + r] = Wt(QV_C1, n, 0, r, 4);
        }
        put_chunk(img.data() + OFF_W1, 64, 0, n, k32);
        put_chunk(img.data() + OFF_W1, 64, 1, n, k32 + 16);
    }
    const int S22[11] = {4, 3, 2, 1, 0, -1, 4, 3, 2, 1, 0};
    const int S3[7] = {2, 1, 0, -1, 2, 1, 0};
    int8_t c16[16];
    for (int s = 0; s < 5; ++s)
        for (int h = 0; h < 2; ++h) {
            uint8_t *blk = img.data() + OFF_W22 + (s * 2 + h) * T22;
            for (int bi = 0; bi < 11; ++bi)
                if (S22[bi] >= 0)
                    for (int j = 0; j < 2; ++j)
                        for (int ch = 0; ch < 16; ++ch) {
                            for (int b = 0; b < 16; ++b) c16[b] = Wt(QV_C2_2, ch, 32 * h + 16 * j + b, S22[bi], s);
                            put_chunk(blk, NR22, j, bi * 16 + ch, c16);
                        }
        }
    for (int s = 0; s < 3; ++s)
        for (int h = 0; h < 2; ++h) {
            uint8_t *blk = img.data() + OFF_W21 + (s * 2 + h) * T21;
            for (int bi = 0; bi < 7; ++bi)
                if (S3[bi] >= 0)
                    for (int j = 0; j < 2; ++j)
                        for (int ch = 0; ch < 32; ++ch) {
                            for (int b = 0; b < 16; ++b) c16[b] = Wt(QV_C2_1, ch, 32 * h + 16 * j + b, S3[bi], s);
                            put_chunk(blk, NR21, j, bi * 32 + ch, c16);
                        }
        }
    auto unit = [](int k, int j, int &s, int &pl) -> bool {
        if (k < 3) { s = k; pl = j; return true; }
        if (k == 3) { s = j; pl = 2; return true; }
        s = 2; pl = 2;
        return j == 0;
    };
    for (int k = 0; k < 5; ++k)
        for (int bi = 0; bi < 7; ++bi)
            if (S3[bi] >= 0)
                for (int j = 0; j < 2; ++j) {
                    int s, pl;
                    if (!unit(k, j, s, pl)) continue;
                    for (int ch = 0; ch < 16; ++ch) {
                        for (int b = 0; b < 16; ++b) c16[b] = Wt(QV_C3_1, ch, 16 * pl + b, S3[bi], s);
                        put_chunk(img.data() + OFF_W31 + k * T31, NR31, j, bi * 16 + ch, c16);
                    }
                }
    for (int ch = 0; ch < 32; ++ch)
        for (int pl = 0; pl < 3; ++pl) {
            for (int b = 0; b < 16; ++b) c16[b] = Wt(QV_C3_2, ch, 16 * pl + b, 0, 0);
            put_chunk(img.data() + OFF_W32 + (pl / 2) * T32, NR32, pl == 2 ? 1 : pl, ch, c16);
        }
    auto mkq = [&](int l, GroupQ &g) -> bool {
        const LayerHost &L = m.L[l];
        g.blu = L.blu; g.mul = L.mul; g.shift = L.shift; g.rbias = (1 << (L.shift - 1)) / L.mul;
        g.hi = L.blu + g.rbias;
        const long long top = ((long long)L.blu + g.rbias) * L.mul;
        const bool ok = L.shift <= 24 && L.mul < (1ll << L.shift) && top < (1ll << 31) && (top >> L.shift) == 127 && g.hi < (1 << 30);
        g.M = ok ? (unsigned)((unsigned long long)L.mul << (24 - L.shift)) : 0u;
        return ok;
    };
    bool fast = true;
    fast &= mkq(QV_C1, P.q1); fast &= mkq(QV_C2_2, P.q22); fast &= mkq(QV_C2_1, P.q21);
    fast &= mkq(QV_C3_1, P.q31); fast &= mkq(QV_C3_2, P.q32);
    int *bias = reinterpret_cast<int *>(img.data() + OFF_BIAS);
    auto addb = [&](int l, int dst0, const GroupQ &g) {
        for (int k = 0; k < kLayers[l].cout; ++k) bias[dst0 + k] = m.L[l].b[k] + (fast ? g.rbias : 0);
    };
    addb(QV_C1, 0, P.q1);
    addb(QV_C2_2, 64, P.q22); addb(QV_C2_1, 64 + 16, P.q21);
    addb(QV_C3_1, 112, P.q31); addb(QV_C3_2, 112 + 16, P.q32);
    memcpy(P.bias, bias, sizeof(P.bias));
    P.c4_bias = m.L[QV_C4].b[0]; P.c4_mul = m.L[QV_C4].mul; P.c4_shift = m.L[QV_C4].shift;
    for (int t = 0; t < 9; ++t)
        for (int pl = 0; pl < 3; ++pl)
            for (int j = 0; j < 4; ++j) {
                unsigned v = 0;
                for (int b = 0; b < 4; ++b) v |= (unsigned)(uint8_t)Wt(QV_C4, 0, 16 * pl + 4 * j + b, t / 3, t % 3) << (8 * b);
                P.c4_w[(t * 3 + pl) * 4 + j] = (int)v;
            }
    return fast;
}

void fused_debug_tables(const ModelHost &m, std::vector<uint8_t> &wimg, std::vector<uint32_t> &ops, std::vector<int32_t> &consts)
{
    FusedParams P{};
    const bool fast = build_host_image(m, wimg, P);
    PhaseBases pb[N_PHASE];
    FixedBases fb;
    build_mma_bases(0, 0, pb, fb);
    std::vector<PhaseOps> po(N_PHASE);
    build_mma_ops(pb, fb, po.data());
    ops.assign(reinterpret_cast<const uint32_t *>(po.data()), reinterpret_cast<const uint32_t *>(po.data() + N_PHASE));
    consts = {WIMG_BYTES, SMEM_BYTES, OFF_A1, OFF_A2, OFF_IM, OFF_ZERO, OFF_IN, OFF_A3, PW, PLANE, A1_ROW, A2_ROW, IM_BYTES, IN_SLOTS,
              IN_PITCH, WT, PIPE, TM_D1, TM_R22, TM_R21, TM_R31, TM_D32, N_PHASE, N_MMA, fast ? 1 : 0, P.c4_bias, P.c4_mul, P.c4_shift};
    for (const GroupQ *g : {&P.q1, &P.q22, &P.q21, &P.q31, &P.q32})
        for (int v : {g->hi, (int)g->M, g->blu, g->mul, g->shift, g->rbias}) consts.push_back(v);
    consts.insert(consts.end(), P.bias, P.bias + BIAS_INTS);
    consts.insert(consts.end(), P.c4_w, P.c4_w + 108);
}

FusedModel *fused_upload(const ModelHost &m, cudaStream_t st)
{
    std::vector<uint8_t> img;
    FusedModel *fm = new FusedModel();
    FusedParams &P = fm->proto;
    fm->fast = build_host_image(m, img, P);
    cudaError_t e = cudaMalloc(&fm->d_wimg, WIMG_BYTES);
    if (e == cudaSuccess) e = cudaMemcpyAsync(fm->d_wimg, img.data(), WIMG_BYTES, cudaMemcpyHostToDevice, st);
    if (e == cudaSuccess) e = cudaStreamSynchronize(st);
    if (e == cudaSuccess) e = cudaFuncSetAttribute(k_fused<true, false, false>, cudaFuncAttributeMaxDynamicSharedMemorySize, SMEM_BYTES);
    if (e == cudaSuccess) e = cudaFuncSetAttribute(k_fused<false, false, false>, cudaFuncAttributeMaxDynamicSharedMemorySize, SMEM_BYTES);
    if (e == cudaSuccess) e = cudaFuncSetAttribute(k_fused<true, false, true>, cudaFuncAttributeMaxDynamicSharedMemorySize, SMEM_BYTES);
    if (e == cudaSuccess) e = cudaFuncSetAttribute(k_fused<false, false, true>, cudaFuncAttributeMaxDynamicSharedMemorySize, SMEM_BYTES);
    if (e == cudaSuccess) e = cudaFuncSetAttribute(k_fused<true, true, false>, cudaFuncAttributeMaxDynamicSharedMemorySize, SMEM_BYTES);
    if (e == cudaSuccess) e = cudaFuncSetAttribute(k_fused<true, false, false, true>, cudaFuncAttributeMaxDynamicSharedMemorySize, SMEM_BYTES_T);
    if (e == cudaSuccess) e = cudaFuncSetAttribute(k_enh_sse<true, false>, cudaFuncAttributeMaxDynamicSharedMemorySize, SMEM_BYTES);
    if (e == cudaSuccess) e = cudaFuncSetAttribute(k_enh_sse<false, false>, cudaFuncAttributeMaxDynamicSharedMemorySize, SMEM_BYTES);
    if (e == cudaSuccess) e = cudaFuncSetAttribute(k_enh_sse<true, true>, cudaFuncAttributeMaxDynamicSharedMemorySize, SMEM_BYTES);
    if (e == cudaSuccess) e = cudaFuncSetAttribute(k_enh_sse<false, true>, cudaFuncAttributeMaxDynamicSharedMemorySize, SMEM_BYTES);
    if (e == cudaSuccess) e = cudaFuncSetAttribute(k_bases, cudaFuncAttributeMaxDynamicSharedMemorySize, SMEM_BYTES);
    int dev = 0, sms = 148;
    if (e == cudaSuccess) e = cudaGetDevice(&dev);
    if (e == cudaSuccess && (dev < 0 || dev >= 64)) e = cudaErrorInvalidDevice;
    if (e == cudaSuccess) {
        std::lock_guard<std::mutex> lock(g_ops_mu);
        OpsRecord &rec = g_ops_done[dev];
        if (!rec.done) {
            uint32_t *d_b = nullptr, h_b[2] = {0, 0};
            e = cudaMalloc(&d_b, 8);
            if (e == cudaSuccess) {
                k_bases<<<1, 32, SMEM_BYTES, st>>>(d_b);
                e = cudaMemcpyAsync(h_b, d_b, 8, cudaMemcpyDeviceToHost, st);
                if (e == cudaSuccess) e = cudaStreamSynchronize(st);
                cudaFree(d_b);
            }
            if (e == cudaSuccess) {
                PhaseBases pb[N_PHASE];
                FixedBases fb;
                build_mma_bases(h_b[0] >> 4, h_b[1], pb, fb);
                std::vector<PhaseOps> ops(N_PHASE);
                build_mma_ops(pb, fb, ops.data());
                e = cudaMemcpyToSymbolAsync(c_ops, ops.data(), sizeof(PhaseOps) * N_PHASE, 0, cudaMemcpyHostToDevice, st);
                if (e == cudaSuccess) e = cudaStreamSynchronize(st);
                if (e == cudaSuccess) { rec.done = true; rec.sbase16 = h_b[0] >> 4; rec.tmem_base = h_b[1]; }
            }
        }
        P.sbase16 = rec.sbase16; P.tmem_base = rec.tmem_base;
    }
    if (e == cudaSuccess) e = cudaDeviceGetAttribute(&sms, cudaDevAttrMultiProcessorCount, dev);
    if (e != cudaSuccess) {
        set_error("fused_upload: %s", cudaGetErrorString(e));
        cudaFree(fm->d_wimg);
        delete fm;
        return nullptr;
    }
    fm->sm_count = sms;
    fm->env_profile = getenv("QV_FUSED_PROFILE") != nullptr;
    fm->env_experiment = getenv("QV_FUSED_EXPERIMENT") ? atoi(getenv("QV_FUSED_EXPERIMENT")) : 0;
    fm->env_test_fail = getenv("QV_FUSED_TEST_FAIL") != nullptr;
    fm->env_tma = getenv("QV_FUSED_TMA") != nullptr && atoi(getenv("QV_FUSED_TMA")) != 0;
    fm->env_linear = !(getenv("QV_FUSED_LINEAR") && atoi(getenv("QV_FUSED_LINEAR")) == 0);
    if (fm->env_tma) {
        cudaDriverEntryPointQueryResult qr;
        if (cudaGetDriverEntryPoint("cuTensorMapEncodeTiled", &fm->encode_tiled, cudaEnableDefault, &qr) != cudaSuccess || qr != cudaDriverEntryPointSuccess)
            fm->encode_tiled = nullptr;
        cudaGetLastError();
    }
    P.wimg = fm->d_wimg;
    P.fail_flag = nullptr;
    if (cudaHostAlloc(&fm->h_fail, sizeof(int), cudaHostAllocMapped) == cudaSuccess) {
        *fm->h_fail = 0;
        if (cudaHostGetDevicePointer(&P.fail_flag, fm->h_fail, 0) != cudaSuccess) P.fail_flag = nullptr;
    }
    if (!P.fail_flag) {
        set_error("fused_upload: no mapped host memory for the failure report");
        if (fm->h_fail) cudaFreeHost(fm->h_fail);
        cudaFree(fm->d_wimg);
        delete fm;
        return nullptr;
    }
    return fm;
}

cudaError_t fused_wait_words(const FusedModel *fm, const uint32_t *a, uint32_t va, const uint32_t *b, uint32_t vb, cudaStream_t st)
{
    if (!a && !b) return cudaSuccess;
    k_wait_words<<<1, 2, 0, st>>>(a, va, b, vb, fm->proto.fail_flag);
    return cudaGetLastError();
}

void fused_free(FusedModel *fm)
{
    if (!fm) return;
    if (fm->h_fail) cudaFreeHost(fm->h_fail);
    cudaFree(fm->d_wimg);
    delete fm;
}

int fused_take_failure(const FusedModel *fm)
{
    if (!fm || !fm->h_fail) return 0;
    const int f = *reinterpret_cast<volatile int *>(fm->h_fail);
    if (f) *fm->h_fail = 0;
    return f;
}

static cudaError_t plan_units(FusedParams &P, int sm_count, bool allow_linear, bool rows_mode, int &grid)
{
    const int rows_out = P.ye - P.ys;
    P.nstrips = (P.W + WT - 1) / WT;
    grid = 1;
    P.linear = 0;
    if (rows_mode) {
        const long long total = (long long)P.nstrips * rows_out;
        if (total > 0x3fffffffll) return cudaErrorInvalidValue;
        grid = (int)std::max<long long>(1, std::min<long long>(sm_count, total / 32));
        P.seg_rows = (int)((total + grid - 1) / grid);
        grid = (int)((total + P.seg_rows - 1) / P.seg_rows);
        const int pieces = (P.seg_rows + rows_out - 1) / rows_out + 1;
        P.nseg = 1;
        P.n_units = grid * pieces;
    } else {
        const long long cols = (long long)P.n_frames * P.nstrips;
        int nseg = 1;
        {
            long long best = -1;
            const int max_seg = std::max(1, std::min(rows_out / 16, 256));
            for (int c = 1; c <= max_seg; ++c) {
                const int rws = (rows_out + c - 1) / c, real = (rows_out + rws - 1) / rws;
                const long long waves = (cols * real + sm_count - 1) / sm_count;
                const long long cost = waves * (rws + PIPE);
                if (best < 0 || cost < best) { best = cost; nseg = c; }
            }
        }
        P.seg_rows = (rows_out + nseg - 1) / nseg;
        P.nseg = (rows_out + P.seg_rows - 1) / P.seg_rows;
        const long long units = cols * P.nseg;
        if (units > 0x7fffffffll) return cudaErrorInvalidValue;
        P.n_units = (int)units;
        grid = (int)std::min<long long>(units, sm_count);
        const long long total = cols * rows_out, g2 = std::max<long long>(1, std::min<long long>(sm_count, total / 32));
        const long long chunk = (total + g2 - 1) / g2, pieces = (chunk + rows_out - 1) / rows_out + 1;
        const long long cost_equal = (units + grid - 1) / grid * (P.seg_rows + PIPE);
        if (allow_linear && total <= 0x3fffffffll && chunk + pieces * PIPE < cost_equal) {
            P.linear = 1;
            P.seg_rows = (int)chunk;
            grid = (int)((total + chunk - 1) / chunk);
            P.nseg = 1;
            P.n_units = grid * (int)pieces;
            const long long per = (cols + grid - 1) / grid;
            P.perm_q = (int)((cols + per - 1) / per);
            P.perm_s0 = (int)(cols / P.perm_q);
            P.perm_r = (int)(cols % P.perm_q);
        }
    }
    return cudaSuccess;
}

int fused_debug_units(int sm_count, int n_frames, int H, int W, int row0, int row1, bool rows_mode, bool allow_linear, std::vector<int> &units, int &grid)
{
    FusedParams P{};
    P.n_frames = n_frames; P.H = H; P.W = W; P.ys = row0; P.ye = row1;
    if (sm_count < 1 || n_frames < 1 || W < 1 || row0 < 0 || row1 > H || row0 >= row1 || (rows_mode && n_frames != 1)) return -1;
    if (plan_units(P, sm_count, allow_linear, rows_mode, grid) != cudaSuccess) return -1;
    units.clear();
    for (int u = 0; u < P.n_units; ++u) {
        const UnitGeo g = rows_mode ? unit_geo<true>(P, u, H, grid) : unit_geo<false>(P, u, H, grid);
        if (!g.ok) continue;
        const int v[5] = {u % grid, g.f, g.strip, g.y0, g.y1};
        units.insert(units.end(), v, v + 5);
    }
    return 0;
}

cudaError_t fused_forward(const FusedModel *fm, const uint8_t *d_in, uint8_t *d_out, int n, int H, int W, cudaStream_t st,
                          long long *launches, const FusedRows *rows, const uint8_t *d_ori, int64_t *d_sse)
{
    if (n <= 0) return cudaSuccess;
    const bool sse = d_ori && d_sse;
    if ((d_ori || d_sse) && !sse) return cudaErrorInvalidValue;
    if (sse && H > FUSED_SSE_MAX_H) return cudaErrorInvalidValue;
    FusedParams P = fm->proto;
    P.ori = d_ori;
    P.sse = reinterpret_cast<unsigned long long *>(d_sse);
    P.n_frames = n; P.H = H; P.W = W;
    P.frame_stride = (size_t)H * W;
    P.in = d_in; P.out = d_out;
    P.ys = P.own0 = P.rlo = 0; P.ye = P.own1 = P.rhi = H;
    P.in_top = P.in_bot = nullptr; P.flag_top = P.flag_bot = nullptr;
    P.pub = P.done = P.done_ctr = nullptr; P.seq = 0;
    if (rows) {
        if (n != 1 || rows->own0 < 0 || rows->own1 > H || rows->own0 >= rows->own1 || rows->out0 < rows->own0 || rows->out1 > rows->own1 ||
            rows->out0 > rows->out1 || rows->top_rows < 0 || rows->bot_rows < 0)
            return cudaErrorInvalidValue;
        if (rows->out0 == rows->out1) return cudaSuccess;
        P.own0 = rows->own0; P.own1 = rows->own1; P.ys = rows->out0; P.ye = rows->out1;
        P.rlo = rows->d_top ? rows->own0 - rows->top_rows : rows->own0;
        P.rhi = rows->d_bot ? rows->own1 + rows->bot_rows : rows->own1;
        if (P.rlo < 0 || P.rhi > H) return cudaErrorInvalidValue;
        P.in = d_in - (ptrdiff_t)rows->own0 * W;
        P.out = d_out - (ptrdiff_t)rows->out0 * W;
        if (sse) P.ori = d_ori - (ptrdiff_t)rows->out0 * W;
        P.in_top = rows->d_top ? rows->d_top - (ptrdiff_t)P.rlo * W : nullptr;
        P.in_bot = rows->d_bot ? rows->d_bot - (ptrdiff_t)rows->own1 * W : nullptr;
        P.flag_top = rows->d_top ? rows->flag_top : nullptr;
        P.flag_bot = rows->d_bot ? rows->flag_bot : nullptr;
        P.pub = rows->pub; P.done = rows->done; P.done_ctr = rows->done_ctr; P.seq = rows->seq;
    }
    int grid = 1;
    if (const cudaError_t e = plan_units(P, fm->sm_count, fm->env_linear, rows != nullptr, grid)) return e;
    const bool prof = fm->env_profile;
    P.dbg = nullptr;
    P.dbg_flags = fm->env_experiment;
    if (fm->env_test_fail) P.sbase16 ^= 1u;
    const size_t dbg_n = (size_t)grid * 16 + TR_N * 48;
    if (prof && !rows && !sse && cudaMalloc(&P.dbg, dbg_n * sizeof(long long)) != cudaSuccess) P.dbg = nullptr;
    if (P.dbg) cudaMemsetAsync(P.dbg, 0, dbg_n * sizeof(long long), st);
    bool tma = false;
    if (fm->env_tma && fm->encode_tiled && !rows && !sse && fm->fast && !P.dbg && W % 16 == 0 && W >= IN_BOX && ((uintptr_t)d_in & 15) == 0) {
        using EncodeFn = CUresult (*)(CUtensorMap *, CUtensorMapDataType, cuuint32_t, void *, const cuuint64_t *, const cuuint64_t *, const cuuint32_t *,
                                      const cuuint32_t *, CUtensorMapInterleave, CUtensorMapSwizzle, CUtensorMapL2promotion, CUtensorMapFloatOOBfill);
        const cuuint64_t dims[2] = {(cuuint64_t)W, (cuuint64_t)n * (cuuint64_t)H}, strides[1] = {(cuuint64_t)W};
        const cuuint32_t box[2] = {(cuuint32_t)IN_BOX, 1}, estr[2] = {1, 1};
        tma = reinterpret_cast<EncodeFn>(fm->encode_tiled)(&P.tmap_in, CU_TENSOR_MAP_DATA_TYPE_UINT8, 2, const_cast<uint8_t *>(d_in), dims, strides, box, estr,
                                                            CU_TENSOR_MAP_INTERLEAVE_NONE, CU_TENSOR_MAP_SWIZZLE_NONE, CU_TENSOR_MAP_L2_PROMOTION_L2_128B,
                                                            CU_TENSOR_MAP_FLOAT_OOB_FILL_NONE) == CUDA_SUCCESS;
    }
    if (sse && rows) {
        if (fm->fast) k_enh_sse<true, true><<<grid, NTHREADS, SMEM_BYTES, st>>>(P);
        else k_enh_sse<false, true><<<grid, NTHREADS, SMEM_BYTES, st>>>(P);
    } else if (sse) {
        if (fm->fast) k_enh_sse<true, false><<<grid, NTHREADS, SMEM_BYTES, st>>>(P);
        else k_enh_sse<false, false><<<grid, NTHREADS, SMEM_BYTES, st>>>(P);
    } else if (tma) k_fused<true, false, false, true><<<grid, NTHREADS, SMEM_BYTES_T, st>>>(P);
    else if (rows && fm->fast) k_fused<true, false, true><<<grid, NTHREADS, SMEM_BYTES, st>>>(P);
    else if (rows) k_fused<false, false, true><<<grid, NTHREADS, SMEM_BYTES, st>>>(P);
    else if (fm->fast && P.dbg) k_fused<true, true, false><<<grid, NTHREADS, SMEM_BYTES, st>>>(P);
    else if (fm->fast) k_fused<true, false, false><<<grid, NTHREADS, SMEM_BYTES, st>>>(P);
    else k_fused<false, false, false><<<grid, NTHREADS, SMEM_BYTES, st>>>(P);
    if (launches) *launches += 1;
    cudaError_t e = cudaGetLastError();
    if (P.dbg) {
        std::vector<long long> h(dbg_n);
        cudaStreamSynchronize(st);
        cudaMemcpy(h.data(), P.dbg, h.size() * sizeof(long long), cudaMemcpyDeviceToHost);
        cudaFree(P.dbg);
        double a[16] = {0};
        for (int b = 0; b < grid; ++b) for (int k = 0; k < 16; ++k) a[k] += (double)h[(size_t)b * 16 + k] / grid;
        const double iters = P.linear ? (double)P.seg_rows + PIPE * (P.n_units / grid - 1) : (double)P.n_units / grid * (P.seg_rows + PIPE);
        fprintf(stderr, "[qv fused profile] units=%d grid=%d iters/block~%.0f | cycles per iteration: MMA warp wait=%.0f issue=%.0f | "
                "worker w0: wait_mma=%.0f drain=%.0f (of which tcgen05.ld+wait %.0f) fence+arrive=%.0f bar=%.0f | "
                "second traced worker (thread NWORKER/2): wait_mma=%.0f drain=%.0f (tcgen05.ld+wait %.0f) fence+arrive=%.0f bar=%.0f\n",
                P.n_units, grid, iters, a[0] / iters, a[1] / iters, a[2] / iters, a[3] / iters, a[14] / iters, a[4] / iters, a[5] / iters,
                a[8] / iters, a[9] / iters, a[15] / iters, a[10] / iters, a[11] / iters);
        const long long *tr = h.data() + (size_t)grid * 16, t0 = tr[0];
        if (t0)
            for (int k = 0; k < TR_N; ++k, tr += 16)
                fprintf(stderr, "[qv fused trace] it %d | mma: start %lld end %lld | w0: commit %lld drained %lld arrived %lld bar %lld | "
                        "w4: commit %lld drained %lld arrived %lld bar %lld\n", TR_ITER0 + k, tr[0] - t0, tr[1] - t0, tr[2] - t0, tr[3] - t0,
                        tr[4] - t0, tr[5] - t0, tr[6] - t0, tr[7] - t0, tr[8] - t0, tr[9] - t0);
        tr = h.data() + (size_t)grid * 16;
        if (t0)
            for (int k = 0; k < TR_N; ++k, tr += 16)
                fprintf(stderr, "[qv fused mma-side] it %d | loop top %lld  wait done %lld  fence done %lld  (issue start %lld)  commit issued %lld  end %lld\n",
                        TR_ITER0 + k, tr[10] - t0, tr[11] - t0, tr[12] - t0, tr[0] - t0, tr[13] - t0, tr[1] - t0);
        if (t0)
            for (int k = 0; k < TR_N; ++k) {
                const long long *sp = h.data() + (size_t)grid * 16 + TR_N * 16 + k * 32, s0 = h[(size_t)grid * 16 + k * 16];
                fprintf(stderr, "[qv fused stamps] it %d:", TR_ITER0 + k);
                for (int j = 0; j < 27; ++j) fprintf(stderr, " %lld", sp[j] - (j ? sp[j - 1] : s0));
                fprintf(stderr, "\n");
            }
    }
    return e;
}

}
```

### qcnn_gpu_b200/csrc/qv_fused.h

```cpp
#pragma once
#include <cstdint>
#include <vector>
#include <cuda_runtime.h>

#include "qv_internal.h"

namespace qv {

struct FusedModel;

FusedModel *fused_upload(const ModelHost &m, cudaStream_t st);
void fused_free(FusedModel *fm);
struct FusedRows {
    int own0 = 0, own1 = 0, out0 = 0, out1 = 0, top_rows = 0, bot_rows = 0;
    const uint8_t *d_top = nullptr, *d_bot = nullptr;
    const uint32_t *flag_top = nullptr, *flag_bot = nullptr;
    uint32_t *pub = nullptr, *done = nullptr, *done_ctr = nullptr;
    uint32_t seq = 0;
};
constexpr int FUSED_SSE_MAX_H = 66051;
cudaError_t fused_forward(const FusedModel *fm, const uint8_t *d_in, uint8_t *d_out, int n, int H, int W,
                          cudaStream_t st, long long *launches, const FusedRows *rows = nullptr,
                          const uint8_t *d_ori = nullptr, int64_t *d_sse = nullptr);
cudaError_t fused_wait_words(const FusedModel *fm, const uint32_t *a, uint32_t va, const uint32_t *b, uint32_t vb, cudaStream_t st);
int fused_take_failure(const FusedModel *fm);

void fused_debug_tables(const ModelHost &m, std::vector<uint8_t> &wimg, std::vector<uint32_t> &ops, std::vector<int32_t> &consts);
int fused_debug_units(int sm_count, int n_frames, int H, int W, int row0, int row1, bool rows_mode, bool allow_linear, std::vector<int> &units, int &grid);

}
```

### qcnn_gpu_b200/csrc/qv_fused_body.inc

```
    static_assert(!(TMA && ROWS), "the TMA input ring exists for whole-frame launches only");
    static_assert(!(SSE && (TMA || PROF)), "no SSE form of the TMA input ring or of the profiling build");
    constexpr int IN_BASE = TMA ? OFF_IN_T : OFF_IN, IN_ROWPITCH = TMA ? IN_PITCH_T : IN_PITCH;
    extern __shared__ __align__(1024) uint8_t sm[];
    uint64_t *bar_mma = reinterpret_cast<uint64_t *>(sm + OFF_CTRL);
    uint32_t *s_tmem = reinterpret_cast<uint32_t *>(sm + OFF_CTRL + 32);
    int *s_fail = reinterpret_cast<int *>(sm + OFF_CTRL + 36);
    const int tid = threadIdx.x, warp = tid >> 5, lane = tid & 31;
    const int H = P.H, W = P.W;

    if (ROWS && P.pub && blockIdx.x == 0 && tid == 0) asm volatile("st.release.sys.global.u32 [%0], %1;" ::"l"(P.pub), "r"(P.seq) : "memory");
#pragma unroll
    for (int j = 0; j < QV_CODE_SHIFT; ++j) asm volatile("membar.cta;" ::: "memory");
#if QV_BULK_WEIGHTS
    static_assert(WIMG_BYTES % 16 == 0 && WIMG_BYTES < (1 << 20), "cp.async.bulk size / mbarrier tx-count");
    uint64_t *bar_in = reinterpret_cast<uint64_t *>(sm + OFF_CTRL + 40);
    uint64_t *bar_w = reinterpret_cast<uint64_t *>(sm + OFF_CTRL + 56);
    if (tid == 0) {
        mbar_init(&bar_mma[0], 1);
        mbar_init(&bar_mma[1], 1);
        if (TMA) { mbar_init(&bar_in[0], 1); mbar_init(&bar_in[1], 1); }
        mbar_init(bar_w, 1);
        *s_fail = 0;
        mbar_fence_init();
        constexpr uint32_t PART = (WIMG_BYTES / 4 + 15) / 16 * 16;
        asm volatile("mbarrier.arrive.expect_tx.shared::cta.b64 _, [%0], %1;" ::"r"(smem_u32(bar_w)), "r"((uint32_t)WIMG_BYTES) : "memory");
#pragma unroll
        for (uint32_t o = 0; o < (uint32_t)WIMG_BYTES; o += PART) {
            const uint32_t n = o + PART <= (uint32_t)WIMG_BYTES ? PART : (uint32_t)WIMG_BYTES - o;
            asm volatile("cp.async.bulk.shared::cluster.global.mbarrier::complete_tx::bytes [%0], [%1], %2, [%3];"
                         ::"r"(smem_u32(sm + o)), "l"(P.wimg + o), "r"(n), "r"(smem_u32(bar_w)) : "memory");
        }
    }
    for (int i = tid; i < (OFF_CTRL - OFF_A1) / 16; i += NTHREADS)
        reinterpret_cast<uint4 *>(sm + OFF_A1)[i] = make_uint4(0, 0, 0, 0);
    if (tid == 0 && !tc::mbar_wait(bar_w, 0)) *s_fail = 1;
#else
    for (int i = tid; i < WIMG_BYTES / 16; i += NTHREADS)
        reinterpret_cast<uint4 *>(sm)[i] = reinterpret_cast<const uint4 *>(P.wimg)[i];
    for (int i = tid; i < (OFF_CTRL - OFF_A1) / 16; i += NTHREADS)
        reinterpret_cast<uint4 *>(sm + OFF_A1)[i] = make_uint4(0, 0, 0, 0);
    uint64_t *bar_in = reinterpret_cast<uint64_t *>(sm + OFF_CTRL + 40);
    if (tid == 0) {
        mbar_init(&bar_mma[0], 1);
        mbar_init(&bar_mma[1], 1);
        if (TMA) { mbar_init(&bar_in[0], 1); mbar_init(&bar_in[1], 1); }
        *s_fail = 0;
        mbar_fence_init();
    }
#endif
    if (warp == MMA_WARP) { tmem_alloc(s_tmem, TM_COLS); tmem_relinquish(); }
    fence_proxy_async_smem();
    fence_before_sync();
    __syncthreads();
    fence_after_sync();
    const uint32_t tm = *s_tmem;
    const uint32_t sbase = smem_u32(sm);

    if (warp == MMA_WARP) {
        const bool leader = elect_one();
        uint32_t nb3 = 0, ev_mma = 0;
        long long t_wait = 0, t_issue = 0, tc0 = PROF ? clock64() : 0;
        const bool issue = leader && !(PROF && (P.dbg_flags & 1));
        long long *stamp = nullptr;
        constexpr std::integral_constant<int, COL_DISCARD> ONCE{};
        constexpr std::integral_constant<int, COL_FILL> KEEP{};
        constexpr std::integral_constant<int, COL_USE> AGAIN{};
        constexpr std::integral_constant<int, COL_LASTUSE> LAST{};
        if ((sbase >> 4) != P.sbase16 || tm != P.tmem_base) { if (lane == 0) *s_fail = 2; }
        const uint32_t r22 = tm + TM_R22, r21 = tm + TM_R21, r31 = tm + TM_R31;
        for (int unit = blockIdx.x; unit < P.n_units; unit += gridDim.x) {
            const UnitGeo g = unit_geo<ROWS>(P, unit, H, (int)gridDim.x);
            if (!g.ok) continue;
            const int y0 = g.y0, y1 = g.y1;
            const int niter = y1 - y0 + PIPE;
            int ph = mod_pos(y0 - 4, N_PHASE);
            for (int i = 0; i < niter; ++i) {
                const PhaseOps &op = c_ops[ph];
                auto MMA = [&](auto col, uint32_t d, int k, uint32_t idesc, uint32_t acc) {
                    const uint4 ab = op.ab[k];
                    if (issue) mma_i8_ss_col<decltype(col)::value>(d, ((uint64_t)ab.y << 32) | ab.x, ((uint64_t)ab.w << 32) | ab.z, idesc, acc);
                    if (PROF && stamp) *stamp++ = clock64();
                };
                asm volatile("bar.sync %0, %1;" ::"r"(2u + nb3), "n"(NWORKER + NC4 + 32) : "memory");
                nb3 = nb3 == 2 ? 0 : nb3 + 1;
                fence_after_sync();
                bool tr = false;
                if (PROF) {
                    const long long t = clock64(); t_wait += t - tc0; tc0 = t;
                    tr = P.dbg && leader && unit == 0 && i >= TR_ITER0 && i < TR_ITER0 + TR_N;
                    if (tr) P.dbg[gridDim.x * 16 + (i - TR_ITER0) * 16 + 0] = tc0;
                    stamp = (tr && !QV_LIGHT_PROF) ? P.dbg + gridDim.x * 16 + TR_N * 16 + (i - TR_ITER0) * 32 : nullptr;
                }
                MMA(ONCE, op.d1, 0, idesc_i8(128, 64), 0);
                MMA(KEEP, op.z22, 1, idesc_i8(128, 16), 0);
                MMA(AGAIN, op.z21, 2, idesc_i8(128, 32), 0);
                MMA(LAST, op.z31, 3, idesc_i8(128, 16), 0);
                MMA(ONCE, r31, 4, idesc_i8(128, 64), 1);
                MMA(KEEP, r31, 5, idesc_i8(128, 64), 1);
                MMA(LAST, op.d32, 6, idesc_i8(128, 32), 0);
                MMA(ONCE, r31, 7, idesc_i8(128, 64), 1);
                MMA(KEEP, r31, 8, idesc_i8(128, 64), 1);
                MMA(LAST, op.d32, 9, idesc_i8(128, 32), 1);
                MMA(ONCE, r31, 10, idesc_i8(128, 64), 1);
                int k = 11;
#pragma unroll
                for (int t = 0; t < 10; ++t) {
                    const int s = t / 2;
                    if (s >= 1 && s <= 3) {
                        MMA(KEEP, r22, k++, idesc_i8(128, 96), 1);
                        MMA(LAST, r21, k++, idesc_i8(128, 128), 1);
                    } else {
                        MMA(ONCE, r22, k++, idesc_i8(128, 96), 1);
                    }
                }
                ph = wrap_inc(ph, N_PHASE);
                if (leader) mma_commit(&bar_mma[ev_mma & 1]);
                ++ev_mma;
                __syncwarp();
                if (PROF) {
                    const long long t = clock64(); t_issue += t - tc0; tc0 = t;
                    if (tr) P.dbg[gridDim.x * 16 + (i - TR_ITER0) * 16 + 1] = tc0;
                }
            }
        }
        if (PROF && P.dbg && leader) { P.dbg[blockIdx.x * 16 + 0] = t_wait; P.dbg[blockIdx.x * 16 + 1] = t_issue; }
    } else if (warp < NWORKER / 32) {
#pragma unroll
        for (int j = 0; j < QV_SHIFT_WORK; ++j) asm volatile("membar.cta;" ::: "memory");
        const int q = warp & 3, hh = warp >> 2;
        const int m = q * 32 + lane;
        const uint32_t tm_lane = tm + ((uint32_t)(q * 32) << 16);
        uint32_t ev_work = 0, ev_mma = 0;
        long long tw[6] = {0, 0, 0, 0, 0, 0}, tc0 = PROF ? clock64() : 0, t_ldtm = 0;
        int tr_slot = -1;
        auto lap = [&](int k) {
            if (PROF && QV_LIGHT_PROF) {
                if (tr_slot >= 0 && k < 4) P.dbg[gridDim.x * 16 + tr_slot + k] = clock64();
            } else if (PROF) {
                const long long t = clock64(); tw[k] += t - tc0; tc0 = t;
                if (tr_slot >= 0 && k < 4) P.dbg[gridDim.x * 16 + tr_slot + k] = t;
            }
        };
        auto worker_bar = []() { asm volatile("bar.sync 1, %0;" ::"n"(NWORKER + NC4) : "memory"); };
        for (int unit = blockIdx.x; unit < P.n_units; unit += gridDim.x) {
            const UnitGeo g = unit_geo<ROWS>(P, unit, H, (int)gridDim.x);
            if (!g.ok) continue;
            const int strip = g.strip, f = g.f, y0 = g.y0, y1 = g.y1;
            const int X0 = strip * WT;
            const int niter = y1 - y0 + PIPE;
            worker_bar();
            work_arrive(ev_work);
            ++ev_work;
            int c3 = mod_pos(y0 - 4, 3), c6 = mod_pos(y0 - 4, 6);
            const bool xa1 = (unsigned)(X0 - 4 + m) < (unsigned)W, xa2 = (unsigned)(X0 - 2 + m) < (unsigned)W, xa3 = (unsigned)(X0 - 1 + m) < (unsigned)W;
            for (int i = 0; i < niter; ++i, c3 = wrap_inc(c3, 3), c6 = wrap_inc(c6, 6)) {
                const int R1 = y0 - 4 + i, R1p = R1 + 4096;
                if (PROF)
                    tr_slot = (P.dbg && unit == 0 && (tid == 0 || tid == NWORKER / 2) && i >= TR_ITER0 && i < TR_ITER0 + TR_N)
                                  ? (i - TR_ITER0) * 16 + 2 + (tid / (NWORKER / 2)) * 4 : -1;
                if (PROF && i >= 1 && (P.dbg_flags & 2)) {
                    warp_wait(&bar_mma[ev_mma & 1], (ev_mma >> 1) & 1, lane, s_fail);
                    ++ev_mma;
                    fence_after_sync();
                    lap(0);
                } else if (i >= 1) {
                    warp_wait(&bar_mma[ev_mma & 1], (ev_mma >> 1) & 1, lane, s_fail);
                    ++ev_mma;
                    fence_after_sync();
                    lap(0);
                    const uint32_t par = (R1p - 1) & 1;
                    auto row_ok = [&](int r) { return (unsigned)r < (unsigned)H; };
                    const bool v1 = row_ok(R1 - 1) && xa1;
                    uint8_t *dst1 = sm + OFF_A1 + wrap_sub(c3, 1, 3) * A1_ROW + (4 + m) * 16;
                    const uint32_t d1 = tm_lane + TM_D1 + par * 64;
                    uint32_t ra[16], rb[16], rc[16], rd[16], re[16];
                    auto drain_a = [&]() {
                        const bool v2 = row_ok(R1 - 5) && xa2, v2n = row_ok(R1 - 4) && xa2, v3 = row_ok(R1 - 8) && xa3;
                        uint8_t *dst2 = sm + OFF_A2 + wrap_sub(c3, 5, 3) * A2_ROW + (6 + m) * 16;
                        uint8_t *dst2n = sm + OFF_A2 + wrap_sub(c3, 4, 3) * A2_ROW + (6 + m) * 16;
                        tmem_ld_x16(d1 + 0, ra); tmem_ld_x16(d1 + 16, rb);
                        tmem_ld_x16(tm_lane + TM_R22 + wrap_sub(c6, 5, 6) * 16, rc);
                        tmem_ld_x16(tm_lane + TM_R21 + ((R1p - 4) & 3) * 32, rd);
                        tmem_ld_x16(tm_lane + TM_R31 + ((R1p - 8) & 3) * 16, re);
                        tmem_ld_wait();
                        requant_store<FAST, 0>(ra, P, P.q1, v1, dst1 + 0 * PLANE);
                        requant_store<FAST, 16>(rb, P, P.q1, v1, dst1 + 1 * PLANE);
                        requant_store<FAST, 64>(rc, P, P.q22, v2, dst2 + 2 * PLANE);
                        requant_store<FAST, 80>(rd, P, P.q21, v2n, dst2n + 0 * PLANE);
                        if (!(EXP & 1)) requant_store<FAST, 112>(re, P, P.q31, v3, sm + OFF_A3 + wrap_sub(c3, 8, 3) * A2_ROW + (7 + m) * 16);
                    };
                    auto drain_b = [&]() {
                        const bool v2n = row_ok(R1 - 4) && xa2, v3n = row_ok(R1 - 7) && xa3;
                        uint8_t *dst2n = sm + OFF_A2 + wrap_sub(c3, 4, 3) * A2_ROW + (6 + m) * 16;
                        const uint32_t d32 = tm_lane + TM_D32 + par * 32;
                        tmem_ld_x16(d1 + 32, ra); tmem_ld_x16(d1 + 48, rb);
                        tmem_ld_x16(tm_lane + TM_R21 + ((R1p - 4) & 3) * 32 + 16, rc);
                        tmem_ld_x16(d32 + 0, rd); tmem_ld_x16(d32 + 16, re);
                        tmem_ld_wait();
                        requant_store<FAST, 32>(ra, P, P.q1, v1, dst1 + 2 * PLANE);
                        requant_store<FAST, 48>(rb, P, P.q1, v1, dst1 + 3 * PLANE);
                        requant_store<FAST, 96>(rc, P, P.q21, v2n, dst2n + 1 * PLANE);
                        if (!(EXP & 1)) {
                            uint8_t *dst3n = sm + OFF_A3 + wrap_sub(c3, 7, 3) * A2_ROW + (7 + m) * 16;
                            requant_store<FAST, 128>(rd, P, P.q32, v3n, dst3n + 1 * PLANE);
                            requant_store<FAST, 144>(re, P, P.q32, v3n, dst3n + 2 * PLANE);
                        }
                    };
#if QV_ONE_WORKER
                    if (FAST) {
                        uint32_t rf[16], rg[16], rh[16], ri[16], rj[16];
                        const bool v2 = row_ok(R1 - 5) && xa2, v2n = row_ok(R1 - 4) && xa2, v3 = row_ok(R1 - 8) && xa3, v3n = row_ok(R1 - 7) && xa3;
                        uint8_t *dst2 = sm + OFF_A2 + wrap_sub(c3, 5, 3) * A2_ROW + (6 + m) * 16;
                        uint8_t *dst2n = sm + OFF_A2 + wrap_sub(c3, 4, 3) * A2_ROW + (6 + m) * 16;
                        uint8_t *dst3n = sm + OFF_A3 + wrap_sub(c3, 7, 3) * A2_ROW + (7 + m) * 16;
                        const uint32_t d32 = tm_lane + TM_D32 + par * 32;
                        tmem_ld_x16(d1 + 0, ra); tmem_ld_x16(d1 + 16, rb); tmem_ld_x16(d1 + 32, rf); tmem_ld_x16(d1 + 48, rg);
                        tmem_ld_x16(tm_lane + TM_R22 + wrap_sub(c6, 5, 6) * 16, rc);
                        tmem_ld_x16(tm_lane + TM_R21 + ((R1p - 4) & 3) * 32, rd);
                        tmem_ld_x16(tm_lane + TM_R21 + ((R1p - 4) & 3) * 32 + 16, rh);
                        tmem_ld_x16(tm_lane + TM_R31 + ((R1p - 8) & 3) * 16, re);
                        tmem_ld_x16(d32 + 0, ri); tmem_ld_x16(d32 + 16, rj);
                        tmem_ld_wait();
                        requant_store<FAST, 0>(ra, P, P.q1, v1, dst1 + 0 * PLANE);
                        requant_store<FAST, 16>(rb, P, P.q1, v1, dst1 + 1 * PLANE);
                        requant_store<FAST, 32>(rf, P, P.q1, v1, dst1 + 2 * PLANE);
                        requant_store<FAST, 48>(rg, P, P.q1, v1, dst1 + 3 * PLANE);
                        requant_store<FAST, 64>(rc, P, P.q22, v2, dst2 + 2 * PLANE);
                        requant_store<FAST, 80>(rd, P, P.q21, v2n, dst2n + 0 * PLANE);
                        requant_store<FAST, 96>(rh, P, P.q21, v2n, dst2n + 1 * PLANE);
                        requant_store<FAST, 112>(re, P, P.q31, v3, sm + OFF_A3 + wrap_sub(c3, 8, 3) * A2_ROW + (7 + m) * 16);
                        requant_store<FAST, 128>(ri, P, P.q32, v3n, dst3n + 1 * PLANE);
                        requant_store<FAST, 144>(rj, P, P.q32, v3n, dst3n + 2 * PLANE);
                    } else {
                        drain_a();
                        drain_b();
                    }
#else
                    if (hh == 0) drain_a(); else drain_b();
#endif
                }
                lap(1);
                if (i + 1 < niter) {
                    fence_proxy_async_smem();
                    fence_before_sync();
                    work_arrive(ev_work);
                    ++ev_work;
                }
                lap(2);
                worker_bar();
                lap(3);
            }
            warp_wait(&bar_mma[ev_mma & 1], (ev_mma >> 1) & 1, lane, s_fail);
            ++ev_mma;
            fence_after_sync();
            worker_bar();
            tr_slot = -1;
            lap(5);
        }
        if (PROF && P.dbg && (tid == 0 || tid == NWORKER / 2))
        {
            for (int k = 0; k < 6; ++k) P.dbg[blockIdx.x * 16 + 2 + (tid / (NWORKER / 2)) * 6 + k] = tw[k];
            P.dbg[blockIdx.x * 16 + 14 + (tid / (NWORKER / 2))] = t_ldtm;
        }
    } else {
#pragma unroll
        for (int j = 0; j < QV_SHIFT_C4; ++j) asm volatile("membar.cta;" ::: "memory");
        const int mo = tid - (NWORKER + 32);
        uint32_t ev_work = 0, tma_n = 0;
        auto worker_bar = []() { asm volatile("bar.sync 1, %0;" ::"n"(NWORKER + NC4) : "memory"); };
        for (int unit = blockIdx.x; unit < P.n_units; unit += gridDim.x) {
            const UnitGeo g = unit_geo<ROWS>(P, unit, H, (int)gridDim.x);
            if (!g.ok) continue;
            const int strip = g.strip, f = g.f, y0 = g.y0, y1 = g.y1;
            const int X0 = strip * WT;
            const int niter = y1 - y0 + PIPE;
            const uint8_t *inf = P.in + (size_t)f * (ROWS ? P.frame_stride : (size_t)H * W);
            uint8_t *outf = P.out + (size_t)f * (ROWS ? P.frame_stride : (size_t)H * W);
            const uint8_t *orif = SSE ? P.ori + (size_t)f * (ROWS ? P.frame_stride : (size_t)H * W) : nullptr;
            const bool col_ok = mo < WT && X0 + mo < W;
            uint32_t sse_in = 0, sse_out = 0;
            const int col_a = X0 - 8 + mo, col_b = col_a + 128;
            const bool ok_a = col_a >= 0 && col_a < W, ok_b = mo < PW - 128 && col_b < W;
            const bool peer_unit = ROWS && ((P.in_top && y0 - 6 < P.own0) || (P.in_bot && y1 + PIPE > P.own1));
            auto load_in = [&](int row) -> unsigned {
                const bool rok = ROWS ? (unsigned)(row - P.rlo) < (unsigned)(P.rhi - P.rlo) : (row >= 0 && row < H);
                const uint8_t *rp = inf + (size_t)row * W;
                if (ROWS && peer_unit) rp = (row < P.own0 ? P.in_top : (row >= P.own1 ? P.in_bot : inf)) + (ptrdiff_t)row * W;
                const unsigned a = (rok && ok_a) ? (unsigned)rp[col_a] : 128u;
                const unsigned b = (rok && ok_b) ? (unsigned)rp[col_b] : 128u;
                return a | (b << 8);
            };
            const int in_sh = TMA ? ((X0 - 8) & 15) : 0;
            auto store_in = [&](int row, unsigned v) {
                uint8_t *rp = sm + IN_BASE + in_sh + ((row + 4096) & (IN_SLOTS - 1)) * IN_ROWPITCH;
                rp[mo] = (uint8_t)v;
                if (mo < PW - 128) rp[128 + mo] = (uint8_t)(v >> 8);
            };
            const bool edge = X0 == 0 || X0 - 8 + PW > W;
            auto tma_expect = [&](int b, uint32_t tx) {
                asm volatile("mbarrier.arrive.expect_tx.shared::cta.b64 _, [%0], %1;" ::"r"(smem_u32(&bar_in[b])), "r"(tx) : "memory");
            };
            auto tma_row = [&](int row, int b) {
                const uint32_t dst = smem_u32(sm + IN_BASE + ((row + 4096) & (IN_SLOTS - 1)) * IN_ROWPITCH);
                asm volatile("cp.async.bulk.tensor.2d.shared::cluster.global.tile.mbarrier::complete_tx::bytes [%0], [%1, {%2, %3}], [%4];"
                             ::"r"(dst), "l"(&P.tmap_in), "r"(X0 - 8 - in_sh), "r"(f * H + row), "r"(smem_u32(&bar_in[b])) : "memory");
            };
            auto patch_edges = [&](int row) {
                uint8_t *rp = sm + IN_BASE + in_sh + ((row + 4096) & (IN_SLOTS - 1)) * IN_ROWPITCH;
                if (!ok_a) rp[mo] = 128;
                if (mo < PW - 128 && col_b >= W) rp[128 + mo] = 128;
            };
            const int m = mo;
            auto im2col = [&](int R, int buf) {
                uint32_t A[5], bcol = 0, b4 = 0;
                const int p = m + 2, o8 = (p & 3) * 8;
#pragma unroll
                for (int r = 0; r < 5; ++r) {
                    const uint32_t *rowp = reinterpret_cast<const uint32_t *>(sm + IN_BASE + in_sh + ((R + 4094 + r) & (IN_SLOTS - 1)) * IN_ROWPITCH) + (p >> 2);
                    const uint32_t w0 = rowp[0], w1 = rowp[1];
                    A[r] = __funnelshift_r(w0, w1, o8);
                    const uint32_t b = (w1 >> o8) & 0xffu;
                    if (r < 4) bcol |= b << (8 * r); else b4 = b;
                }
                uint8_t *dst = sm + OFF_IM + buf * IM_BYTES + m * 16;
                *reinterpret_cast<uint4 *>(dst) = make_uint4(A[0] ^ 0x80808080u, A[1] ^ 0x80808080u, A[2] ^ 0x80808080u, A[3] ^ 0x80808080u);
                *reinterpret_cast<uint4 *>(dst + 128 * 16) = make_uint4(A[4] ^ 0x80808080u, bcol ^ 0x80808080u, b4 ^ 0x80u, 0u);
            };
            int c3 = mod_pos(y0 - 4, 3);
            int c4_s1 = 0, c4_s2 = 0;
            if (ROWS && P.flag_top && y0 - 6 < P.own0 && P.rlo < P.own0) { if (lane == 0 && !peer_wait(P.flag_top, P.seq)) *s_fail = 3; __syncwarp(); }
            if (ROWS && P.flag_bot && y1 + PIPE > P.own1 && P.rhi > P.own1) { if (lane == 0 && !peer_wait(P.flag_bot, P.seq)) *s_fail = 3; __syncwarp(); }
            if (TMA) {
                const int r_lo = max(y0 - 6, 0), r_hi = min(y0, H);
                if (r_hi > r_lo) {
                    if (mo == 0) {
                        fence_proxy_async_smem();
                        tma_expect(tma_n & 1, (uint32_t)(r_hi - r_lo) * IN_BOX);
                        for (int r = r_lo; r < r_hi; ++r) tma_row(r, tma_n & 1);
                    }
                    warp_wait(&bar_in[tma_n & 1], (tma_n >> 1) & 1, lane, s_fail);
                    ++tma_n;
                    if (edge) for (int r = r_lo; r < r_hi; ++r) patch_edges(r);
                }
                for (int r = y0 - 6; r < y0; ++r) if (r < 0 || r >= H) store_in(r, 128u | (128u << 8));
            } else {
                for (int r = y0 - 6; r <= y0 - 1; ++r) store_in(r, load_in(r));
            }
            worker_bar();
            im2col(y0 - 4, c3);
            fence_proxy_async_smem();
            work_arrive(ev_work);
            ++ev_work;
            for (int i = 0; i < niter; ++i, c3 = wrap_inc(c3, 3)) {
                const int R1 = y0 - 4 + i, R1p = R1 + 4096;
                const bool row_in = (unsigned)(R1 + 4) < (unsigned)H;
                unsigned in_next = 128u | (128u << 8);
                const bool out_row = i >= 3 && R1 - 10 >= y0 && R1 - 10 < y1 && col_ok;
                const int ori_x = SSE && out_row ? (int)orif[(size_t)(R1 - 10) * W + X0 + mo] : 0;
                if (TMA) {
                    if (row_in && mo == 0) { tma_expect(tma_n & 1, IN_BOX); tma_row(R1 + 4, tma_n & 1); }
                } else {
                    in_next = load_in(R1 + 4);
                }
                if (i + 1 < niter) {
                    if (!(EXP & 4)) im2col(R1 + 1, wrap_inc(c3, 3));
                    fence_proxy_async_smem();
                    work_arrive(ev_work);
                    ++ev_work;
                }
                if (!(EXP & 1) && !(PROF && (P.dbg_flags & 2)) && i >= 3) {
                    const uint8_t *row = sm + OFF_A3 + c3 * A2_ROW + (7 + mo) * 16;
                    int acc[3] = {0, 0, 0};
                    uint4 v[3];
#pragma unroll
                    for (int pl = 0; pl < 3; ++pl) v[pl] = *reinterpret_cast<const uint4 *>(row + pl * PLANE);
                    c4_taps<0>(v, P, acc);
#pragma unroll
                    for (int pl = 0; pl < 3; ++pl) v[pl] = *reinterpret_cast<const uint4 *>(row + pl * PLANE + 16);
                    c4_taps<1>(v, P, acc);
#pragma unroll
                    for (int pl = 0; pl < 3; ++pl) v[pl] = *reinterpret_cast<const uint4 *>(row + pl * PLANE + 32);
                    c4_taps<2>(v, P, acc);
                    const int u4 = c4_s2 + acc[2];
                    c4_s2 = c4_s1 + acc[1];
                    c4_s1 = acc[0];
                    const int rowo = R1 - 10;
                    if (rowo >= y0 && rowo < y1 && col_ok) {
                        const int x = sm[IN_BASE + in_sh + ((R1p - 10) & (IN_SLOTS - 1)) * IN_ROWPITCH + 8 + mo];
                        const int rec = residual_apply(u4 + P.c4_bias, x, P.c4_mul, P.c4_shift);
                        outf[(size_t)rowo * W + X0 + mo] = (uint8_t)rec;
                        if (SSE) {
                            const int d_in = x - ori_x, d_out = rec - ori_x;
                            sse_in += (uint32_t)(d_in * d_in);
                            sse_out += (uint32_t)(d_out * d_out);
                        }
                    }
                }
                if (TMA && row_in) {
                    warp_wait(&bar_in[tma_n & 1], (tma_n >> 1) & 1, lane, s_fail);
                    ++tma_n;
                    if (edge) patch_edges(R1 + 4);
                } else {
                    store_in(R1 + 4, in_next);
                }
                worker_bar();
            }
            if (SSE) {
                unsigned long long a = sse_in, b = sse_out;
#pragma unroll
                for (int o = 16; o > 0; o >>= 1) { a += __shfl_xor_sync(0xffffffffu, a, o); b += __shfl_xor_sync(0xffffffffu, b, o); }
                if (lane == 0) { atomicAdd(&P.sse[2 * f], a); atomicAdd(&P.sse[2 * f + 1], b); }
            }
            worker_bar();
        }
    }
    fence_before_sync();
    __syncthreads();
    if (warp == MMA_WARP) tmem_dealloc(tm, TM_COLS);
    if (tid == 0 && *s_fail) {
        *reinterpret_cast<volatile int *>(P.fail_flag) = *s_fail;
        __threadfence_system();
    }
    if (ROWS && P.done && tid == 0) {
        __threadfence();
        if (atomicAdd(P.done_ctr, 1u) == gridDim.x - 1) {
            *P.done_ctr = 0;
            asm volatile("st.release.sys.global.u32 [%0], %1;" ::"l"(P.done), "r"(P.seq) : "memory");
        }
    }
    if (tid == 0 && *s_fail == 3) printf("qv fused kernel: block %d waited in vain for a neighbour GPU's rows (step %u)\n", blockIdx.x, P.seq);
    else if (tid == 0 && *s_fail)
        printf(*s_fail == 2 ? "qv fused kernel: block %d has other shared-memory / TMEM bases than the descriptor table was built for\n"
                            : "qv fused kernel: mbarrier wait timed out in block %d\n", blockIdx.x);
```

Before: 21420.

## Add merged C3 MMA kernel variant issuing 25 instead of 27 MMAs per phase

Adds a k_enh25 kernel variant that packs the C3_1 and C3_2 weight tiles into one combined shared-memory tile. This lets the paired C3_1 and C3_2 MMAs run as a single N=96 instruction, and C1 becomes an N=96 MMA against a zero-padded weight tile. The goal is to cut the number of tcgen05 MMA issues and commit boundaries per row phase. In exchange it needs a second weight image, extra shared memory, a reshuffled TMEM column layout and a separate constant-memory op table. Wider MMAs also compute some padded columns that are thrown away.

Result: slower. 20860 (median of 6 runs) (-2.6%).

```diff
diff --git a/include/qvrcnn_b200.h b/include/qvrcnn_b200.h
--- a/include/qvrcnn_b200.h
+++ b/include/qvrcnn_b200.h
@@ -90,6 +90,7 @@
 QV_API int qv_get_activation(qv_net *net, int which , int8_t *host_out);
 
 QV_API int qv_debug_fused_tables(const void *model_image, size_t len, uint8_t *wimg, uint32_t *ops, int32_t *consts, size_t sizes[3]);
+QV_API int qv_debug_fused_tables25(const void *model_image, size_t len, uint8_t *wimg, uint32_t *ops, int32_t *consts, size_t sizes[3]);
 
 QV_API int qv_debug_fused_units(int sm_count, int n_frames, int height, int width, int row0, int row1, int row_window, int allow_line,
                                 int32_t *units, size_t *n_units, int *grid);
diff --git a/qcnn_gpu_b200/api.py b/qcnn_gpu_b200/api.py
--- a/qcnn_gpu_b200/api.py
+++ b/qcnn_gpu_b200/api.py
@@ -20,7 +20,7 @@
     "qv_set_impl", "qv_get_impl", "qv_launch_count", "qv_get_activation",
     "qv_convert_model_hwcn_to_vect_c", "qv_yuv_read_luma", "qv_yuv_read_frame", "qv_yuv_write_recon",
     "qv_psnr", "qv_psnr_from_sse", "qv_solve_quant_params", "qv_write_quant_params_cpp", "qv_quantize_layer",
-    "qv_debug_fused_tables", "qv_debug_fused_units", "qv_synchronize",
+    "qv_debug_fused_tables", "qv_debug_fused_tables25", "qv_debug_fused_units", "qv_synchronize",
     "qv_strip_setup", "qv_strip_export", "qv_strip_attach", "qv_strip_input", "qv_strip_acquire", "qv_strip_load",
     "qv_strip_forward", "qv_strip_forward_sse", "qv_strip_release",
 )
diff --git a/qcnn_gpu_b200/csrc/qv_api.cu b/qcnn_gpu_b200/csrc/qv_api.cu
--- a/qcnn_gpu_b200/csrc/qv_api.cu
+++ b/qcnn_gpu_b200/csrc/qv_api.cu
@@ -302,7 +302,7 @@
     return sync_model(net);
 }
 
-int qv_debug_fused_tables(const void *image, size_t len, uint8_t *wimg, uint32_t *ops, int32_t *consts, size_t sizes[3])
+static int debug_fused_tables(bool merge3, const void *image, size_t len, uint8_t *wimg, uint32_t *ops, int32_t *consts, size_t sizes[3])
 {
     if (!image || !sizes) { set_error("qv_debug_fused_tables: null argument"); return QV_ERR_ARG; }
     ModelHost m;
@@ -311,12 +311,22 @@
     std::vector<uint8_t> w;
     std::vector<uint32_t> o;
     std::vector<int32_t> c;
-    fused_debug_tables(m, w, o, c);
+    fused_debug_tables(m, merge3, w, o, c);
     if (wimg && sizes[0] >= w.size()) memcpy(wimg, w.data(), w.size());
     if (ops && sizes[1] >= o.size()) memcpy(ops, o.data(), o.size() * sizeof(uint32_t));
     if (consts && sizes[2] >= c.size()) memcpy(consts, c.data(), c.size() * sizeof(int32_t));
     sizes[0] = w.size(); sizes[1] = o.size(); sizes[2] = c.size();
     return QV_OK;
+}
+
+int qv_debug_fused_tables(const void *image, size_t len, uint8_t *wimg, uint32_t *ops, int32_t *consts, size_t sizes[3])
+{
+    return debug_fused_tables(false, image, len, wimg, ops, consts, sizes);
+}
+
+int qv_debug_fused_tables25(const void *image, size_t len, uint8_t *wimg, uint32_t *ops, int32_t *consts, size_t sizes[3])
+{
+    return debug_fused_tables(true, image, len, wimg, ops, consts, sizes);
 }
 
 int qv_debug_fused_units(int sm_count, int n_frames, int height, int width, int row0, int row1, int row_window, int allow_line,
diff --git a/qcnn_gpu_b200/csrc/qv_fused.cu b/qcnn_gpu_b200/csrc/qv_fused.cu
--- a/qcnn_gpu_b200/csrc/qv_fused.cu
+++ b/qcnn_gpu_b200/csrc/qv_fused.cu
@@ -70,6 +70,13 @@
 constexpr int OFF_IN_T = (SMEM_BYTES + 127) / 128 * 128;
 constexpr int SMEM_BYTES_T = OFF_IN_T + IN_SLOTS * IN_PITCH_T;
 static_assert(SMEM_BYTES_T <= 232448, "exceeds the 227 KB of dynamic shared memory per CTA");
+constexpr int NR3M = 64 + 32 + 64, T3M = 2 * NR3M * 16;
+constexpr int W3M_BYTES = 4 * T3M;
+constexpr int OFF_W3M = (SMEM_BYTES + 127) / 128 * 128;
+constexpr int SMEM_BYTES_25 = OFF_W3M + W3M_BYTES;
+constexpr int NR1M = 32 + 64 + 32, OFF_W1M = OFF_W31 + T31, W1M_LBO = 2 * T31;
+static_assert(NR1M * 16 <= T31, "a K-chunk of the C1 tile fits in the place of a C3_1 tile");
+static_assert(SMEM_BYTES_25 <= 232448, "exceeds the 227 KB of dynamic shared memory per CTA");
 
 #ifndef QV_ONE_WORKER
 #define QV_ONE_WORKER 1
@@ -84,6 +91,7 @@
 constexpr int TM_R21 = 224;
 constexpr int TM_R31 = 352;
 constexpr int TM_D32 = 416;
+constexpr int TM_D1_25 = 0, D1_25_STEP = 192, TM_D32_25 = 64, TM_R31_25 = 96, D32_25_STEP = 96, TM_R22_25 = 256, TM_R21_25 = 352;
 constexpr int TM_COLS = 512;
 
 struct GroupQ {
@@ -119,16 +127,27 @@
 struct PhaseBases {
     uint32_t im, a1_r2, a2_r6, b22;
     uint32_t b21, b31, d1, d32;
-    uint32_t z22, z21, z31, pad;
+    uint32_t z22, z21, z31, b3m;
+    uint32_t b1;
 };
 struct FixedBases { uint32_t zeroA, w1, w32, r22, r21, r31, pad0, pad1; };
 constexpr int N_PHASE = 12;
-constexpr int N_MMA = 27;
-struct PhaseOps {
-    uint4 ab[N_MMA];
+constexpr int N_MMA = 27, N_MMA_25 = 25;
+template <int N>
+struct PhaseOpsN {
+    uint4 ab[N];
     uint32_t d1, d32, z22, z21, z31, pad[3];
 };
+using PhaseOps = PhaseOpsN<N_MMA>;
+using PhaseOps25 = PhaseOpsN<N_MMA_25>;
 __constant__ PhaseOps c_ops[N_PHASE];
+__constant__ PhaseOps25 c_ops25[N_PHASE];
+template <bool MERGE3>
+__device__ __forceinline__ const auto &phase_ops(int ph)
+{
+    if constexpr (MERGE3) return c_ops25[ph];
+    else return c_ops[ph];
+}
 
 __host__ __device__ __forceinline__ int mod_pos(int a, int m) { int r = a % m; return r < 0 ? r + m : r; }
 
@@ -244,14 +263,21 @@
 template <bool FAST, bool PROF, bool ROWS, bool TMA = false>
 __global__ void __launch_bounds__(NTHREADS, 1) k_fused(const __grid_constant__ FusedParams P)
 {
-    constexpr bool SSE = false;
+    constexpr bool SSE = false, MERGE3 = false;
 #include "qv_fused_body.inc"
 }
 
 template <bool FAST, bool ROWS>
 __global__ void __launch_bounds__(NTHREADS, 1) k_enh_sse(const __grid_constant__ FusedParams P)
 {
-    constexpr bool SSE = true, PROF = false, TMA = false;
+    constexpr bool SSE = true, PROF = false, TMA = false, MERGE3 = false;
+#include "qv_fused_body.inc"
+}
+
+template <bool FAST>
+__global__ void __launch_bounds__(NTHREADS, 1) k_enh25(const __grid_constant__ FusedParams P)
+{
+    constexpr bool SSE = false, PROF = false, ROWS = false, TMA = false, MERGE3 = true;
 #include "qv_fused_body.inc"
 }
 
@@ -277,16 +303,18 @@
     tmem_dealloc(tm, TM_COLS);
 }
 
-void build_mma_bases(uint32_t sb, uint32_t tm, PhaseBases *pb, FixedBases &fb)
+void build_mma_bases(uint32_t sb, uint32_t tm, bool merge3, PhaseBases *pb, FixedBases &fb)
 {
     constexpr uint32_t LP = (uint32_t)(PLANE >> 4) << 16;
     const uint32_t w22 = sb + (OFF_W22 >> 4) + ((uint32_t)NR22 << 16), w21 = sb + (OFF_W21 >> 4) + ((uint32_t)NR21 << 16);
-    const uint32_t w31 = sb + (OFF_W31 >> 4) + ((uint32_t)NR31 << 16);
+    const uint32_t w31 = sb + (OFF_W31 >> 4) + ((uint32_t)NR31 << 16), w3m = sb + (OFF_W3M >> 4) + ((uint32_t)NR3M << 16);
+    const uint32_t tm31 = tm + (merge3 ? TM_R31_25 : TM_R31), tm22 = tm + (merge3 ? TM_R22_25 : TM_R22), tm21 = tm + (merge3 ? TM_R21_25 : TM_R21);
+    const uint32_t w1m = sb + (OFF_W1M >> 4) + ((uint32_t)(W1M_LBO >> 4) << 16);
     fb = FixedBases{};
     fb.zeroA = sb + (OFF_ZERO >> 4) + ((128u * 16 >> 4) << 16);
     fb.w1 = sb + (OFF_W1 >> 4) + (64u << 16);
     fb.w32 = sb + (OFF_W32 >> 4) + ((uint32_t)NR32 << 16);
-    fb.r22 = tm + TM_R22; fb.r21 = tm + TM_R21; fb.r31 = tm + TM_R31;
+    fb.r22 = tm22; fb.r21 = tm21; fb.r31 = tm31;
     for (int ph = 0; ph < N_PHASE; ++ph) {
         const int R1p = ph + 4096 / N_PHASE * N_PHASE + N_PHASE, c3 = ph % 3, c6 = ph % 6;
         const uint32_t par = ph & 1;
@@ -299,31 +327,45 @@
         e.b22 = w22 + (qa <= 2 ? 2 - qa : 8 - qa) * 16;
         e.b21 = w21 + ((1 - (R1p - 2)) & 3) * 32;
         e.b31 = w31 + ((1 - (R1p - 6)) & 3) * 16;
-        e.d1 = tm + TM_D1 + par * 64; e.d32 = tm + TM_D32 + par * 32;
-        e.z22 = tm + TM_R22 + c6 * 16;
-        e.z21 = tm + TM_R21 + ((R1p - 1) & 3) * 32;
-        e.z31 = tm + TM_R31 + ((R1p - 5) & 3) * 16;
-    }
-}
-
-void build_mma_ops(const PhaseBases *pb, const FixedBases &fb, PhaseOps *ops)
-{
+        e.d1 = merge3 ? (par ? tm + TM_D32_25 + D32_25_STEP : tm + TM_D1_25) : tm + TM_D1 + par * 64;
+        e.d32 = merge3 ? (par ? tm31 : tm + TM_D32_25) : tm + TM_D32 + par * 32;
+        e.b1 = merge3 ? w1m + (par ? 0 : 32) : sb + (OFF_W1 >> 4) + (64u << 16);
+        e.z22 = tm22 + c6 * 16;
+        e.z21 = tm21 + ((R1p - 1) & 3) * 32;
+        e.z31 = tm31 + ((R1p - 5) & 3) * 16;
+        e.b3m = w3m + ((R1p & 3) >> 1) * (T3M >> 4) + (par ? 0 : 64);
+    }
+}
+
+template <int N>
+void build_mma_ops(const PhaseBases *pb, const FixedBases &fb, PhaseOpsN<N> *ops)
+{
+    static_assert(N == N_MMA || N == N_MMA_25, "two MMA lists");
+    constexpr bool merge3 = N == N_MMA_25;
     constexpr uint32_t HI = (128u >> 4) | (1u << 14);
     constexpr uint32_t LP = (uint32_t)(PLANE >> 4) << 16, LX = 1u << 16;
     for (int ph = 0; ph < N_PHASE; ++ph) {
         const PhaseBases &e = pb[ph];
-        PhaseOps &o = ops[ph];
-        o = PhaseOps{};
+        PhaseOpsN<N> &o = ops[ph];
+        o = PhaseOpsN<N>{};
         int k = 0;
         auto put = [&](uint32_t a, uint32_t b) { o.ab[k++] = make_uint4(a, HI, b, HI); };
-        put(e.im, fb.w1);
+        put(e.im, e.b1);
         put(fb.zeroA, fb.w1); put(fb.zeroA, fb.w1); put(fb.zeroA, fb.w1);
         put(e.a2_r6 + 6 + LP, e.b31);
-        put(e.a2_r6 + 7 + LP, e.b31 + (T31 >> 4));
-        put(e.a2_r6 + 7 + LP, fb.w32);
+        if (merge3) {
+            put(e.a2_r6 + 7 + LP, e.b3m);
+        } else {
+            put(e.a2_r6 + 7 + LP, e.b31 + (T31 >> 4));
+            put(e.a2_r6 + 7 + LP, fb.w32);
+        }
         put(e.a2_r6 + 8 + LP, e.b31 + 2 * (T31 >> 4));
-        put(e.a2_r6 + ((2 * PLANE) >> 4) + 6 + LX, e.b31 + 3 * (T31 >> 4));
-        put(e.a2_r6 + ((2 * PLANE) >> 4) + 6 + LX, fb.w32 + (T32 >> 4));
+        if (merge3) {
+            put(e.a2_r6 + ((2 * PLANE) >> 4) + 6 + LX, e.b3m + 2 * (T3M >> 4));
+        } else {
+            put(e.a2_r6 + ((2 * PLANE) >> 4) + 6 + LX, e.b31 + 3 * (T31 >> 4));
+            put(e.a2_r6 + ((2 * PLANE) >> 4) + 6 + LX, fb.w32 + (T32 >> 4));
+        }
         put(e.a2_r6 + ((2 * PLANE) >> 4) + 8 + LX, e.b31 + 4 * (T31 >> 4));
         for (int t = 0; t < 10; ++t) {
             const int sft = t / 2, h = t & 1;
@@ -339,7 +381,7 @@
 
 struct FusedModel {
     int *h_fail = nullptr;
-    uint8_t *d_wimg = nullptr;
+    uint8_t *d_wimg = nullptr, *d_wimg25 = nullptr;
     FusedParams proto{};
     bool fast = true;
     int sm_count = 148;
@@ -354,9 +396,9 @@
 
 static void put_chunk(uint8_t *blk, int NR, int j, int n, const int8_t *src16) { memcpy(blk + ((size_t)j * NR + n) * 16, src16, 16); }
 
-static bool build_host_image(const ModelHost &m, std::vector<uint8_t> &img, FusedParams &P)
-{
-    img.assign(WIMG_BYTES, 0);
+static bool build_host_image(const ModelHost &m, bool merge3, std::vector<uint8_t> &img, FusedParams &P)
+{
+    img.assign(WIMG_BYTES + (merge3 ? W3M_BYTES : 0), 0);
     auto Wt = [&](int l, int k, int c, int r, int s) -> int8_t {
         const LayerShape &sh = kLayers[l];
         return m.L[l].w[(((size_t)k * sh.cin + c) * sh.k + r) * sh.k + s];
@@ -416,6 +458,22 @@
         for (int pl = 0; pl < 3; ++pl) {
             for (int b = 0; b < 16; ++b) c16[b] = Wt(QV_C3_2, ch, 16 * pl + b, 0, 0);
             put_chunk(img.data() + OFF_W32 + (pl / 2) * T32, NR32, pl == 2 ? 1 : pl, ch, c16);
+        }
+    for (int kk = 0; kk < 2 && merge3; ++kk)
+        for (int t = 0; t < 2; ++t) {
+            uint8_t *dst = img.data() + WIMG_BYTES + (2 * kk + t) * T3M;
+            const uint8_t *w31 = img.data() + OFF_W31 + (2 * kk + 1) * T31, *w32 = img.data() + OFF_W32 + kk * T32;
+            for (int j = 0; j < 2; ++j) {
+                memcpy(dst + (j * NR3M + 0) * 16, w31 + (j * NR31 + (2 - 2 * t) * 16) * 16, 64 * 16);
+                memcpy(dst + (j * NR3M + 64) * 16, w32 + j * NR32 * 16, NR32 * 16);
+                memcpy(dst + (j * NR3M + 96) * 16, w31 + (j * NR31 + (3 - 2 * t) * 16) * 16, 64 * 16);
+            }
+        }
+    if (merge3)
+        for (int j = 0; j < 2; ++j) {
+            uint8_t *dst = img.data() + OFF_W1M + j * W1M_LBO;
+            memset(dst, 0, NR1M * 16);
+            memcpy(dst + 32 * 16, img.data() + OFF_W1 + j * 64 * 16, 64 * 16);
         }
     auto mkq = [&](int l, GroupQ &g) -> bool {
         const LayerHost &L = m.L[l];
@@ -448,32 +506,43 @@
     return fast;
 }
 
-void fused_debug_tables(const ModelHost &m, std::vector<uint8_t> &wimg, std::vector<uint32_t> &ops, std::vector<int32_t> &consts)
+void fused_debug_tables(const ModelHost &m, bool merge3, std::vector<uint8_t> &wimg, std::vector<uint32_t> &ops, std::vector<int32_t> &consts)
 {
     FusedParams P{};
-    const bool fast = build_host_image(m, wimg, P);
+    const bool fast = build_host_image(m, merge3, wimg, P);
     PhaseBases pb[N_PHASE];
     FixedBases fb;
-    build_mma_bases(0, 0, pb, fb);
-    std::vector<PhaseOps> po(N_PHASE);
-    build_mma_ops(pb, fb, po.data());
-    ops.assign(reinterpret_cast<const uint32_t *>(po.data()), reinterpret_cast<const uint32_t *>(po.data() + N_PHASE));
-    consts = {WIMG_BYTES, SMEM_BYTES, OFF_A1, OFF_A2, OFF_IM, OFF_ZERO, OFF_IN, OFF_A3, PW, PLANE, A1_ROW, A2_ROW, IM_BYTES, IN_SLOTS,
-              IN_PITCH, WT, PIPE, TM_D1, TM_R22, TM_R21, TM_R31, TM_D32, N_PHASE, N_MMA, fast ? 1 : 0, P.c4_bias, P.c4_mul, P.c4_shift};
+    build_mma_bases(0, 0, merge3, pb, fb);
+    if (merge3) {
+        std::vector<PhaseOps25> po(N_PHASE);
+        build_mma_ops(pb, fb, po.data());
+        ops.assign(reinterpret_cast<const uint32_t *>(po.data()), reinterpret_cast<const uint32_t *>(po.data() + N_PHASE));
+    } else {
+        std::vector<PhaseOps> po(N_PHASE);
+        build_mma_ops(pb, fb, po.data());
+        ops.assign(reinterpret_cast<const uint32_t *>(po.data()), reinterpret_cast<const uint32_t *>(po.data() + N_PHASE));
+    }
+    consts = {WIMG_BYTES, merge3 ? SMEM_BYTES_25 : SMEM_BYTES, OFF_A1, OFF_A2, OFF_IM, OFF_ZERO, OFF_IN, OFF_A3, PW, PLANE, A1_ROW, A2_ROW,
+              IM_BYTES, IN_SLOTS, IN_PITCH, WT, PIPE, merge3 ? TM_D1_25 : TM_D1, merge3 ? TM_R22_25 : TM_R22, merge3 ? TM_R21_25 : TM_R21, merge3 ? TM_R31_25 : TM_R31, merge3 ? TM_D32_25 : TM_D32, N_PHASE,
+              merge3 ? N_MMA_25 : N_MMA, fast ? 1 : 0, P.c4_bias, P.c4_mul, P.c4_shift};
     for (const GroupQ *g : {&P.q1, &P.q22, &P.q21, &P.q31, &P.q32})
         for (int v : {g->hi, (int)g->M, g->blu, g->mul, g->shift, g->rbias}) consts.push_back(v);
     consts.insert(consts.end(), P.bias, P.bias + BIAS_INTS);
     consts.insert(consts.end(), P.c4_w, P.c4_w + 108);
+    if (merge3) consts.insert(consts.end(), {OFF_W3M, D32_25_STEP, D1_25_STEP});
 }
 
 FusedModel *fused_upload(const ModelHost &m, cudaStream_t st)
 {
-    std::vector<uint8_t> img;
+    std::vector<uint8_t> img, img25;
     FusedModel *fm = new FusedModel();
     FusedParams &P = fm->proto;
-    fm->fast = build_host_image(m, img, P);
-    cudaError_t e = cudaMalloc(&fm->d_wimg, WIMG_BYTES);
-    if (e == cudaSuccess) e = cudaMemcpyAsync(fm->d_wimg, img.data(), WIMG_BYTES, cudaMemcpyHostToDevice, st);
+    fm->fast = build_host_image(m, false, img, P);
+    build_host_image(m, true, img25, P);
+    cudaError_t e = cudaMalloc(&fm->d_wimg, img.size());
+    if (e == cudaSuccess) e = cudaMalloc(&fm->d_wimg25, img25.size());
+    if (e == cudaSuccess) e = cudaMemcpyAsync(fm->d_wimg, img.data(), img.size(), cudaMemcpyHostToDevice, st);
+    if (e == cudaSuccess) e = cudaMemcpyAsync(fm->d_wimg25, img25.data(), img25.size(), cudaMemcpyHostToDevice, st);
     if (e == cudaSuccess) e = cudaStreamSynchronize(st);
     if (e == cudaSuccess) e = cudaFuncSetAttribute(k_fused<true, false, false>, cudaFuncAttributeMaxDynamicSharedMemorySize, SMEM_BYTES);
     if (e == cudaSuccess) e = cudaFuncSetAttribute(k_fused<false, false, false>, cudaFuncAttributeMaxDynamicSharedMemorySize, SMEM_BYTES);
@@ -485,6 +554,7 @@
     if (e == cudaSuccess) e = cudaFuncSetAttribute(k_enh_sse<false, false>, cudaFuncAttributeMaxDynamicSharedMemorySize, SMEM_BYTES);
     if (e == cudaSuccess) e = cudaFuncSetAttribute(k_enh_sse<true, true>, cudaFuncAttributeMaxDynamicSharedMemorySize, SMEM_BYTES);
     if (e == cudaSuccess) e = cudaFuncSetAttribute(k_enh_sse<false, true>, cudaFuncAttributeMaxDynamicSharedMemorySize, SMEM_BYTES);
+    if (e == cudaSuccess) e = cudaFuncSetAttribute(k_enh25<true>, cudaFuncAttributeMaxDynamicSharedMemorySize, SMEM_BYTES_25);
     if (e == cudaSuccess) e = cudaFuncSetAttribute(k_bases, cudaFuncAttributeMaxDynamicSharedMemorySize, SMEM_BYTES);
     int dev = 0, sms = 148;
     if (e == cudaSuccess) e = cudaGetDevice(&dev);
@@ -504,10 +574,15 @@
             if (e == cudaSuccess) {
                 PhaseBases pb[N_PHASE];
                 FixedBases fb;
-                build_mma_bases(h_b[0] >> 4, h_b[1], pb, fb);
+                build_mma_bases(h_b[0] >> 4, h_b[1], false, pb, fb);
                 std::vector<PhaseOps> ops(N_PHASE);
                 build_mma_ops(pb, fb, ops.data());
                 e = cudaMemcpyToSymbolAsync(c_ops, ops.data(), sizeof(PhaseOps) * N_PHASE, 0, cudaMemcpyHostToDevice, st);
+                PhaseBases pb25[N_PHASE];
+                build_mma_bases(h_b[0] >> 4, h_b[1], true, pb25, fb);
+                std::vector<PhaseOps25> ops25(N_PHASE);
+                build_mma_ops(pb25, fb, ops25.data());
+                if (e == cudaSuccess) e = cudaMemcpyToSymbolAsync(c_ops25, ops25.data(), sizeof(PhaseOps25) * N_PHASE, 0, cudaMemcpyHostToDevice, st);
                 if (e == cudaSuccess) e = cudaStreamSynchronize(st);
                 if (e == cudaSuccess) { rec.done = true; rec.sbase16 = h_b[0] >> 4; rec.tmem_base = h_b[1]; }
             }
@@ -518,6 +593,7 @@
     if (e != cudaSuccess) {
         set_error("fused_upload: %s", cudaGetErrorString(e));
         cudaFree(fm->d_wimg);
+        cudaFree(fm->d_wimg25);
         delete fm;
         return nullptr;
     }
@@ -543,6 +619,7 @@
         set_error("fused_upload: no mapped host memory for the failure report");
         if (fm->h_fail) cudaFreeHost(fm->h_fail);
         cudaFree(fm->d_wimg);
+        cudaFree(fm->d_wimg25);
         delete fm;
         return nullptr;
     }
@@ -561,6 +638,7 @@
     if (!fm) return;
     if (fm->h_fail) cudaFreeHost(fm->h_fail);
     cudaFree(fm->d_wimg);
+    cudaFree(fm->d_wimg25);
     delete fm;
 }
 
@@ -703,7 +781,10 @@
     else if (rows && fm->fast) k_fused<true, false, true><<<grid, NTHREADS, SMEM_BYTES, st>>>(P);
     else if (rows) k_fused<false, false, true><<<grid, NTHREADS, SMEM_BYTES, st>>>(P);
     else if (fm->fast && P.dbg) k_fused<true, true, false><<<grid, NTHREADS, SMEM_BYTES, st>>>(P);
-    else if (fm->fast) k_fused<true, false, false><<<grid, NTHREADS, SMEM_BYTES, st>>>(P);
+    else if (fm->fast) {
+        P.wimg = fm->d_wimg25;
+        k_enh25<true><<<grid, NTHREADS, SMEM_BYTES_25, st>>>(P);
+    }
     else k_fused<false, false, false><<<grid, NTHREADS, SMEM_BYTES, st>>>(P);
     if (launches) *launches += 1;
     cudaError_t e = cudaGetLastError();
diff --git a/qcnn_gpu_b200/csrc/qv_fused.h b/qcnn_gpu_b200/csrc/qv_fused.h
--- a/qcnn_gpu_b200/csrc/qv_fused.h
+++ b/qcnn_gpu_b200/csrc/qv_fused.h
@@ -25,7 +25,7 @@
 cudaError_t fused_wait_words(const FusedModel *fm, const uint32_t *a, uint32_t va, const uint32_t *b, uint32_t vb, cudaStream_t st);
 int fused_take_failure(const FusedModel *fm);
 
-void fused_debug_tables(const ModelHost &m, std::vector<uint8_t> &wimg, std::vector<uint32_t> &ops, std::vector<int32_t> &consts);
+void fused_debug_tables(const ModelHost &m, bool merge3, std::vector<uint8_t> &wimg, std::vector<uint32_t> &ops, std::vector<int32_t> &consts);
 int fused_debug_units(int sm_count, int n_frames, int H, int W, int row0, int row1, bool rows_mode, bool allow_linear, std::vector<int> &units, int &grid);
 
 }
diff --git a/qcnn_gpu_b200/csrc/qv_fused_body.inc b/qcnn_gpu_b200/csrc/qv_fused_body.inc
--- a/qcnn_gpu_b200/csrc/qv_fused_body.inc
+++ b/qcnn_gpu_b200/csrc/qv_fused_body.inc
@@ -1,5 +1,9 @@
     static_assert(!(TMA && ROWS), "the TMA input ring exists for whole-frame launches only");
     static_assert(!(SSE && (TMA || PROF)), "no SSE form of the TMA input ring or of the profiling build");
+    static_assert(!(MERGE3 && (SSE || PROF || ROWS || TMA)), "the five-MMA layer 3 exists for plain whole-frame launches only");
+    constexpr int TM_C31 = MERGE3 ? TM_R31_25 : TM_R31, TM_C22 = MERGE3 ? TM_R22_25 : TM_R22, TM_C21 = MERGE3 ? TM_R21_25 : TM_R21;
+    constexpr int TM_C1 = MERGE3 ? TM_D1_25 : TM_D1, C1_STEP = MERGE3 ? D1_25_STEP : 64;
+    constexpr int TM_C32 = MERGE3 ? TM_D32_25 : TM_D32, C32_STEP = MERGE3 ? D32_25_STEP : 32;
     constexpr int IN_BASE = TMA ? OFF_IN_T : OFF_IN, IN_ROWPITCH = TMA ? IN_PITCH_T : IN_PITCH;
     extern __shared__ __align__(1024) uint8_t sm[];
     uint64_t *bar_mma = reinterpret_cast<uint64_t *>(sm + OFF_CTRL);
@@ -23,13 +27,16 @@
         *s_fail = 0;
         mbar_fence_init();
         constexpr uint32_t PART = (WIMG_BYTES / 4 + 15) / 16 * 16;
-        asm volatile("mbarrier.arrive.expect_tx.shared::cta.b64 _, [%0], %1;" ::"r"(smem_u32(bar_w)), "r"((uint32_t)WIMG_BYTES) : "memory");
+        asm volatile("mbarrier.arrive.expect_tx.shared::cta.b64 _, [%0], %1;" ::"r"(smem_u32(bar_w)), "r"((uint32_t)WIMG_BYTES + (MERGE3 ? W3M_BYTES : 0)) : "memory");
 #pragma unroll
         for (uint32_t o = 0; o < (uint32_t)WIMG_BYTES; o += PART) {
             const uint32_t n = o + PART <= (uint32_t)WIMG_BYTES ? PART : (uint32_t)WIMG_BYTES - o;
             asm volatile("cp.async.bulk.shared::cluster.global.mbarrier::complete_tx::bytes [%0], [%1], %2, [%3];"
                          ::"r"(smem_u32(sm + o)), "l"(P.wimg + o), "r"(n), "r"(smem_u32(bar_w)) : "memory");
         }
+        if (MERGE3)
+            asm volatile("cp.async.bulk.shared::cluster.global.mbarrier::complete_tx::bytes [%0], [%1], %2, [%3];"
+                         ::"r"(smem_u32(sm + OFF_W3M)), "l"(P.wimg + WIMG_BYTES), "r"((uint32_t)W3M_BYTES), "r"(smem_u32(bar_w)) : "memory");
     }
     for (int i = tid; i < (OFF_CTRL - OFF_A1) / 16; i += NTHREADS)
         reinterpret_cast<uint4 *>(sm + OFF_A1)[i] = make_uint4(0, 0, 0, 0);
@@ -37,6 +44,9 @@
 #else
     for (int i = tid; i < WIMG_BYTES / 16; i += NTHREADS)
         reinterpret_cast<uint4 *>(sm)[i] = reinterpret_cast<const uint4 *>(P.wimg)[i];
+    if (MERGE3)
+        for (int i = tid; i < W3M_BYTES / 16; i += NTHREADS)
+            reinterpret_cast<uint4 *>(sm + OFF_W3M)[i] = reinterpret_cast<const uint4 *>(P.wimg + WIMG_BYTES)[i];
     for (int i = tid; i < (OFF_CTRL - OFF_A1) / 16; i += NTHREADS)
         reinterpret_cast<uint4 *>(sm + OFF_A1)[i] = make_uint4(0, 0, 0, 0);
     uint64_t *bar_in = reinterpret_cast<uint64_t *>(sm + OFF_CTRL + 40);
@@ -67,7 +77,7 @@
         constexpr std::integral_constant<int, COL_USE> AGAIN{};
         constexpr std::integral_constant<int, COL_LASTUSE> LAST{};
         if ((sbase >> 4) != P.sbase16 || tm != P.tmem_base) { if (lane == 0) *s_fail = 2; }
-        const uint32_t r22 = tm + TM_R22, r21 = tm + TM_R21, r31 = tm + TM_R31;
+        const uint32_t r22 = tm + TM_C22, r21 = tm + TM_C21, r31 = tm + TM_C31;
         for (int unit = blockIdx.x; unit < P.n_units; unit += gridDim.x) {
             const UnitGeo g = unit_geo<ROWS>(P, unit, H, (int)gridDim.x);
             if (!g.ok) continue;
@@ -75,7 +85,7 @@
             const int niter = y1 - y0 + PIPE;
             int ph = mod_pos(y0 - 4, N_PHASE);
             for (int i = 0; i < niter; ++i) {
-                const PhaseOps &op = c_ops[ph];
+                const auto &op = phase_ops<MERGE3>(ph);
                 auto MMA = [&](auto col, uint32_t d, int k, uint32_t idesc, uint32_t acc) {
                     const uint4 ab = op.ab[k];
                     if (issue) mma_i8_ss_col<decltype(col)::value>(d, ((uint64_t)ab.y << 32) | ab.x, ((uint64_t)ab.w << 32) | ab.z, idesc, acc);
@@ -91,18 +101,26 @@
                     if (tr) P.dbg[gridDim.x * 16 + (i - TR_ITER0) * 16 + 0] = tc0;
                     stamp = (tr && !QV_LIGHT_PROF) ? P.dbg + gridDim.x * 16 + TR_N * 16 + (i - TR_ITER0) * 32 : nullptr;
                 }
-                MMA(ONCE, op.d1, 0, idesc_i8(128, 64), 0);
+                MMA(ONCE, op.d1, 0, idesc_i8(128, MERGE3 ? 96 : 64), 0);
                 MMA(KEEP, op.z22, 1, idesc_i8(128, 16), 0);
                 MMA(AGAIN, op.z21, 2, idesc_i8(128, 32), 0);
                 MMA(LAST, op.z31, 3, idesc_i8(128, 16), 0);
-                MMA(ONCE, r31, 4, idesc_i8(128, 64), 1);
-                MMA(KEEP, r31, 5, idesc_i8(128, 64), 1);
-                MMA(LAST, op.d32, 6, idesc_i8(128, 32), 0);
-                MMA(ONCE, r31, 7, idesc_i8(128, 64), 1);
-                MMA(KEEP, r31, 8, idesc_i8(128, 64), 1);
-                MMA(LAST, op.d32, 9, idesc_i8(128, 32), 1);
-                MMA(ONCE, r31, 10, idesc_i8(128, 64), 1);
-                int k = 11;
+                if constexpr (!MERGE3) {
+                    MMA(ONCE, r31, 4, idesc_i8(128, 64), 1);
+                    MMA(KEEP, r31, 5, idesc_i8(128, 64), 1);
+                    MMA(LAST, op.d32, 6, idesc_i8(128, 32), 0);
+                    MMA(ONCE, r31, 7, idesc_i8(128, 64), 1);
+                    MMA(KEEP, r31, 8, idesc_i8(128, 64), 1);
+                    MMA(LAST, op.d32, 9, idesc_i8(128, 32), 1);
+                    MMA(ONCE, r31, 10, idesc_i8(128, 64), 1);
+                } else {
+                    MMA(ONCE, r31, 4, idesc_i8(128, 64), 1);
+                    MMA(ONCE, op.d32, 5, idesc_i8(128, 96), 1);
+                    MMA(ONCE, r31, 6, idesc_i8(128, 64), 1);
+                    MMA(ONCE, op.d32, 7, idesc_i8(128, 96), 1);
+                    MMA(ONCE, r31, 8, idesc_i8(128, 64), 1);
+                }
+                int k = MERGE3 ? 9 : 11;
 #pragma unroll
                 for (int t = 0; t < 10; ++t) {
                     const int s = t / 2;
@@ -172,16 +190,16 @@
                     auto row_ok = [&](int r) { return (unsigned)r < (unsigned)H; };
                     const bool v1 = row_ok(R1 - 1) && xa1;
                     uint8_t *dst1 = sm + OFF_A1 + wrap_sub(c3, 1, 3) * A1_ROW + (4 + m) * 16;
-                    const uint32_t d1 = tm_lane + TM_D1 + par * 64;
+                    const uint32_t d1 = tm_lane + TM_C1 + par * C1_STEP;
                     uint32_t ra[16], rb[16], rc[16], rd[16], re[16];
                     auto drain_a = [&]() {
                         const bool v2 = row_ok(R1 - 5) && xa2, v2n = row_ok(R1 - 4) && xa2, v3 = row_ok(R1 - 8) && xa3;
                         uint8_t *dst2 = sm + OFF_A2 + wrap_sub(c3, 5, 3) * A2_ROW + (6 + m) * 16;
                         uint8_t *dst2n = sm + OFF_A2 + wrap_sub(c3, 4, 3) * A2_ROW + (6 + m) * 16;
                         tmem_ld_x16(d1 + 0, ra); tmem_ld_x16(d1 + 16, rb);
-                        tmem_ld_x16(tm_lane + TM_R22 + wrap_sub(c6, 5, 6) * 16, rc);
-                        tmem_ld_x16(tm_lane + TM_R21 + ((R1p - 4) & 3) * 32, rd);
-                        tmem_ld_x16(tm_lane + TM_R31 + ((R1p - 8) & 3) * 16, re);
+                        tmem_ld_x16(tm_lane + TM_C22 + wrap_sub(c6, 5, 6) * 16, rc);
+                        tmem_ld_x16(tm_lane + TM_C21 + ((R1p - 4) & 3) * 32, rd);
+                        tmem_ld_x16(tm_lane + TM_C31 + ((R1p - 8) & 3) * 16, re);
                         tmem_ld_wait();
                         requant_store<FAST, 0>(ra, P, P.q1, v1, dst1 + 0 * PLANE);
                         requant_store<FAST, 16>(rb, P, P.q1, v1, dst1 + 1 * PLANE);
@@ -192,9 +210,9 @@
                     auto drain_b = [&]() {
                         const bool v2n = row_ok(R1 - 4) && xa2, v3n = row_ok(R1 - 7) && xa3;
                         uint8_t *dst2n = sm + OFF_A2 + wrap_sub(c3, 4, 3) * A2_ROW + (6 + m) * 16;
-                        const uint32_t d32 = tm_lane + TM_D32 + par * 32;
+                        const uint32_t d32 = tm_lane + TM_C32 + par * C32_STEP;
                         tmem_ld_x16(d1 + 32, ra); tmem_ld_x16(d1 + 48, rb);
-                        tmem_ld_x16(tm_lane + TM_R21 + ((R1p - 4) & 3) * 32 + 16, rc);
+                        tmem_ld_x16(tm_lane + TM_C21 + ((R1p - 4) & 3) * 32 + 16, rc);
                         tmem_ld_x16(d32 + 0, rd); tmem_ld_x16(d32 + 16, re);
                         tmem_ld_wait();
                         requant_store<FAST, 32>(ra, P, P.q1, v1, dst1 + 2 * PLANE);
@@ -213,12 +231,12 @@
                         uint8_t *dst2 = sm + OFF_A2 + wrap_sub(c3, 5, 3) * A2_ROW + (6 + m) * 16;
                         uint8_t *dst2n = sm + OFF_A2 + wrap_sub(c3, 4, 3) * A2_ROW + (6 + m) * 16;
                         uint8_t *dst3n = sm + OFF_A3 + wrap_sub(c3, 7, 3) * A2_ROW + (7 + m) * 16;
-                        const uint32_t d32 = tm_lane + TM_D32 + par * 32;
+                        const uint32_t d32 = tm_lane + TM_C32 + par * C32_STEP;
                         tmem_ld_x16(d1 + 0, ra); tmem_ld_x16(d1 + 16, rb); tmem_ld_x16(d1 + 32, rf); tmem_ld_x16(d1 + 48, rg);
-                        tmem_ld_x16(tm_lane + TM_R22 + wrap_sub(c6, 5, 6) * 16, rc);
-                        tmem_ld_x16(tm_lane + TM_R21 + ((R1p - 4) & 3) * 32, rd);
-                        tmem_ld_x16(tm_lane + TM_R21 + ((R1p - 4) & 3) * 32 + 16, rh);
-                        tmem_ld_x16(tm_lane + TM_R31 + ((R1p - 8) & 3) * 16, re);
+                        tmem_ld_x16(tm_lane + TM_C22 + wrap_sub(c6, 5, 6) * 16, rc);
+                        tmem_ld_x16(tm_lane + TM_C21 + ((R1p - 4) & 3) * 32, rd);
+                        tmem_ld_x16(tm_lane + TM_C21 + ((R1p - 4) & 3) * 32 + 16, rh);
+                        tmem_ld_x16(tm_lane + TM_C31 + ((R1p - 8) & 3) * 16, re);
                         tmem_ld_x16(d32 + 0, ri); tmem_ld_x16(d32 + 16, rj);
                         tmem_ld_wait();
                         requant_store<FAST, 0>(ra, P, P.q1, v1, dst1 + 0 * PLANE);
```
